# taconite/IntrinsicAvatar

Measured on AMD Instinct MI355X. Metric: rays/sec (fwd+bwd) at 540×540, 1024 spp; fraction of HBM / MFMA roofline, higher is better.
Workload: dtype f32

## Files before the change

include/ia_amd.h:

```cpp
#ifndef IA_AMD_H
#define IA_AMD_H

#include <stdint.h>

#ifdef __cplusplus
extern "C" {
#endif

#define IA_OK 0
#define IA_ERR_INVALID (-1)
#define IA_ERR_LAUNCH (-2)
#define IA_ERR_UNSUPPORTED (-3)

typedef void* ia_stream_t;

int ia_version(void);
const char* ia_last_error(void);

int64_t ia_scan_tmp_bytes(int64_t n);
int ia_exclusive_scan_i64(const int64_t* in, int64_t* out, int64_t* total, int64_t n, void* tmp, ia_stream_t stream);
int ia_exclusive_scan_i32(const int32_t* in, int32_t* out, int32_t* total, int64_t n, void* tmp, ia_stream_t stream);

int ia_occgrid_pack_bits(const uint8_t* binaries, int64_t n_cells, uint32_t* bits, ia_stream_t stream);

// ... 55 lines not shown
int ia_ray_resampling(int64_t n_rays, int64_t n_in, int n, const int32_t* packed_info, const float* starts, const float* ends,
                      const float* weights, const float* sdfs, const int32_t* resample_packed_info, int64_t n_out,
                      float* resample_ts, float* resample_offsets, int64_t* surface_idx,
                      int64_t* resample_indices, int32_t* resample_fg_counts, int32_t* resample_bg_counts, void* tmp,
                      ia_stream_t stream);
int ia_ray_resampling_upto(int64_t n_rays, int64_t n_in, int n, const int32_t* packed_info, const float* starts, const float* ends,
                           const float* weights, const float* sdfs, const int32_t* resample_packed_info, int64_t n_out,
                           const int32_t* n_out_dev, float* resample_ts, float* resample_offsets, int64_t* surface_idx,
                           int64_t* resample_indices, int32_t* resample_fg_counts, int32_t* resample_bg_counts, void* tmp,
                           ia_stream_t stream);
int ia_ray_resampling_merge(int64_t n_rays, int64_t n_in, int n, const int32_t* packed_info, const float* vals,
                            const uint8_t* is_left, const uint8_t* is_right, const float* weights,
                            const int32_t* resample_packed_info, float* resample_vals, float* resample_dists,
                            uint8_t* resample_is_left, uint8_t* resample_is_right, uint8_t* is_resample,
                            uint8_t* is_fg_sample, void* tmp, ia_stream_t stream);
int ia_ray_resampling_merge_count(int64_t n_rays, int64_t n_in, int n, const int32_t* packed_info, const float* vals,
                                  const uint8_t* is_left, const uint8_t* is_right, const float* weights, int32_t* cnt,
                                  int32_t* start, int32_t* total, void* tmp, void* scan_tmp, ia_stream_t stream);
int ia_ray_resampling_merge_fill(int64_t n_rays, int64_t n_in, int n, const int32_t* packed_info, const float* vals,
                                 const uint8_t* is_left, const uint8_t* is_right, const int32_t* cnt, const int32_t* start,
                                 float* out_vals, uint8_t* out_is_left, uint8_t* out_is_right, int64_t* out_ray_indices,
                                 int32_t* out_packed_info, void* tmp, ia_stream_t stream);
int ia_ray_resampling_fine(int64_t n_rays, int64_t n_in, int n, const int32_t* packed_info, const float* starts, const float* ends,
                           const float* weights, const int32_t* resample_packed_info, int64_t n_out, float* resample_starts,
                           float* resample_ends, uint8_t* is_fg_sample, void* tmp, ia_stream_t stream);
int ia_ray_resampling_sdf_fine(int64_t n_rays, int64_t n_in, int n, const int32_t* packed_info, const float* starts,
                               const float* ends, const float* alphas, const float* sdfs,
                               const int32_t* resample_packed_info, int64_t n_out, float* resample_starts,
                               float* resample_ends, uint8_t* is_fg_sample, void* tmp, ia_stream_t stream);

int ia_fg_count(int64_t n_rays, const int32_t* resampled_packed_info, const uint8_t* is_fg, int32_t* cnt, int32_t* start, int32_t* total,
                void* scan_tmp, ia_stream_t stream);
int ia_fg_compact(int64_t n_rays, const int32_t* resampled_packed_info, const uint8_t* is_fg, const float* starts, const float* ends,
                  const int32_t* cnt, const int32_t* start, int64_t* ray_indices, float* t_starts, float* t_ends, int32_t* out_packed_info,
                  ia_stream_t stream);

int ia_interval_samples_count(int64_t n_edges, const uint8_t* is_left, int32_t* pos, int32_t* total, void* scan_tmp, ia_stream_t stream);
int ia_interval_samples_count_upto(int64_t capacity, const uint8_t* is_left, const int32_t* n_edges, int32_t* pos, int32_t* total,
                                   void* scan_tmp, ia_stream_t stream);
int ia_interval_samples_fill(int64_t n_rays, int64_t n_edges, const int32_t* edge_packed_info, const float* vals,
                             const int64_t* ray_indices, const uint8_t* is_left, const int32_t* pos, const int32_t* total,
                             int64_t* left_idx, float* t_starts, float* t_ends, int64_t* sample_ray_indices,
                             int32_t* sample_packed_info, ia_stream_t stream);
int ia_samples_to_edges(int64_t n_edges, const uint8_t* is_left, const int32_t* pos, const float* sample_vals, float fill, float* out,
                        ia_stream_t stream);

#define IA_LAYOUT_NCDHW 0
#define IA_LAYOUT_NDHWC 1
int ia_precompute(int B, int D, int H, int W, const float* voxel_w , const float* tfs ,
                  const float* offset , const float* scale ,
                  float* voxel_d , float* voxel_J ,
                  float* voxel_J_cl , ia_stream_t stream);
int ia_fuse_broyden(int B, int64_t N, int I, const float* xd_tgt , const float* voxel_J, int layout,
                    int D, int H, int W, const float* tfs, const int32_t* bone_ids ,
                    const float* offset, const float* scale, float cvg_threshold, float dvg_threshold,
                    float* x , float* J_inv , uint8_t* is_valid ,
                    float* fwd_J ,
                    ia_stream_t stream);
int ia_filter(int64_t N, int I, const float* x , const uint8_t* mask, uint8_t* out, ia_stream_t stream);
int ia_cell_tightness(int D, int H, int W, const float* voxel_J_cl , const float* offset, const float* scale, float tau,
                      uint8_t* cell_tight , ia_stream_t stream);
int ia_fuse_broyden_spec(int64_t N, int I, const float* xd_tgt , const float* voxel_J_cl , int D, int H, int W,
                         const float* tfs , const int32_t* bone_ids, const float* offset, const float* scale,
                         float cvg_threshold, float dvg_threshold, float eps, float* x , float* J_inv ,
                         uint8_t* is_valid , float* fwd_J , uint64_t* counters,
                         const uint8_t* cell_tight , ia_stream_t stream);
int ia_spec_rows_slots(void);
size_t ia_spec_rows_overflow_bytes(int64_t N);
int64_t ia_spec_rows_overflow_capacity(int64_t N);
int ia_fuse_broyden_spec_rows(int64_t N, int I, const float* xd_tgt, const float* voxel_J_cl, int D, int H, int W, const float* tfs,
                              const int32_t* bone_ids, const float* offset, const float* scale, float cvg_threshold,
                              float dvg_threshold, float eps, float* x_rows, float* J_inv, float* fwd_J, int32_t* cnt, uint32_t* meta,
                              int32_t* start, int32_t* ovf_head, void* ovf_scratch, int32_t* total_and_overflow, void* scan_tmp,
                              uint64_t* counters, const int32_t* order ,
                              const uint8_t* cell_tight , ia_stream_t stream);
int ia_deform_rows_pack(int64_t N, int I, const float* x_rows, const int32_t* cnt, const uint32_t* meta, const int32_t* start,
                        const int32_t* ovf_head, const void* ovf_scratch, float* cand_x, int32_t* cand_src,
                        const float* norm_center , const float* norm_scale ,
                        ia_stream_t stream);
int64_t ia_deform_rows_pack_split_tmp_bytes(int64_t N);
int ia_deform_rows_pack_split(int64_t N, int I, const float* x_rows, const int32_t* cnt, const uint32_t* meta, const int32_t* start,
                              const int32_t* ovf_head, const void* ovf_scratch, int32_t* first_pos, int32_t* first_tile_off, int32_t* n_first,
                              float* cand_x, const float* norm_center, const float* norm_scale, void* scan_tmp, ia_stream_t stream);
int ia_deform_select_min_split(int64_t P, const int32_t* start, const int32_t* cnt, const int32_t* first_pos, const int32_t* first_tile_off,
                               const int32_t* n_first, const float* cand_sdf, const int32_t* order, float* sdf, ia_stream_t stream);
int ia_broyden_stats(int B, int64_t N, int I, const float* xd_tgt, const float* voxel_J, int layout, int D, int H, int W,
                     const float* tfs, const int32_t* bone_ids, const float* offset, const float* scale,
                     float cvg_threshold, float dvg_threshold, uint64_t* counters, ia_stream_t stream);
int ia_broyden_voxel_stats(int64_t N, int I, int init_major, const float* xd_tgt, const float* voxel_J , int D, int H,
                           int W, const float* tfs, const int32_t* bone_ids, const float* offset, const float* scale,
                           uint64_t* counters, ia_stream_t stream);

int64_t ia_hashgrid_n_entries(int n_levels, int log2_hashmap_size, int base_resolution, float per_level_scale);
int ia_hashgrid_fwd(int64_t n, const float* x , const float* params, int n_levels, int n_features,
                    int log2_hashmap_size, int base_resolution, float per_level_scale,
                    float* out, int out_stride, float* dy_dx , ia_stream_t stream);
int64_t ia_hashgrid_fwd_scratch_bytes(int64_t n, int n_levels, int with_jac);
int ia_hashgrid_fwd_xcd(int64_t n, const float* x, const float* params, int n_levels, int n_features,
                        int log2_hashmap_size, int base_resolution, float per_level_scale, float* out, int out_stride,
                        float* dy_dx, void* scratch, ia_stream_t stream);
int ia_hashgrid_bwd(int64_t n, const float* x, int n_levels, int n_features, int log2_hashmap_size,
                    int base_resolution, float per_level_scale, const float* g_enc ,
                    int g_enc_stride, const float* g_jac , int g_jac_stride, const float* q ,
                    float* grad_params, ia_stream_t stream);
int64_t ia_hashgrid_bwd_scratch_bytes(int64_t n, int n_levels, int log2_hashmap_size, int base_resolution,
                                      float per_level_scale);
int ia_hashgrid_bwd_binned(int64_t n, const float* x, int n_levels, int n_features, int log2_hashmap_size,
                           int base_resolution, float per_level_scale, const float* g_enc, int g_enc_stride,
                           const float* g_jac, int g_jac_stride, const float* q, float* grad_params,
                           uint32_t level_mask ,
                           void* scratch, int64_t scratch_bytes, ia_stream_t stream);
int ia_hashgrid_jac_contract(int mode, int64_t n, int K, const float* jac, const float* v, int v_stride, float* out,
                             int out_stride, ia_stream_t stream);
int ia_sh4_fwd(int64_t n, const float* d01, float* out, int out_stride, ia_stream_t stream);

int ia_mlp_fwd(int kind, int64_t n, int n_segs, const float* const* seg_ptr, const int* seg_stride,
               const int* seg_width, const float* seg_mul, const float* seg_add,
               const float* W1, const float* b1, const float* W2, const float* b2, const float* Wo, const float* bo,
               float* y, int y_stride, const float* jac, int xyz_col, const float* inv_scale_host, float* grad,
               ia_stream_t stream);

int ia_deform_filter_count(int64_t P, int I, const float* x , const uint8_t* valid ,
                           uint8_t* mask , int32_t* cnt , ia_stream_t stream);
int ia_deform_compact(int64_t P, int I, const float* x, const uint8_t* mask, const int32_t* start,
                      float* cand_x , int32_t* cand_src , ia_stream_t stream);
size_t ia_deform_filter_compact_tmp_bytes(int64_t P);
int ia_deform_filter_compact(int64_t P, int I, const float* x, const uint8_t* valid, int32_t* cnt , int32_t* start ,
                             float* cand_x , int32_t* cand_src , uint8_t* mask ,
                             int32_t* total , void* tmp, size_t tmp_bytes, ia_stream_t stream);
size_t ia_deform_filter_tiles_tmp_bytes(int64_t P);
int ia_deform_filter_tiles(int64_t P, int I, float* x, const uint8_t* valid, int32_t* cnt, int32_t* start, int32_t* src_local ,
                           uint8_t* mask , int32_t* total, void* tmp, size_t tmp_bytes, ia_stream_t stream);
int ia_deform_pack_tiles(int64_t P, int I, const float* x, const int32_t* src_local , int32_t* start, float* cand_x,
                         int32_t* cand_src , const void* tmp, ia_stream_t stream);
int ia_deform_select(int64_t P, const int32_t* start, const int32_t* cnt, const float* cand_x,
                     const int32_t* cand_src, const float* cand_sdf, int sdf_stride, const float* cand_grad ,
                     const float* cand_feat , int feat_stride, int feat_dim, const float* c2w ,
                     float* pts_cano , float* sdf , uint8_t* valid , int32_t* sel ,
                     float* grad_posed , float* grad_cano , float* feat ,
                     ia_stream_t stream);
int ia_ray_points(int64_t n, const float* rays_o, const float* rays_d, const int64_t* ray_indices,
                  const float* t0, const float* t1, float* pts, ia_stream_t stream);
int ia_shade_prep(int64_t n, const float* sdf_grad , const float* rays_d, const int64_t* ray_indices,
                  const float* w2s_rot , float* normal_smpl, float* normal_world, float* refl01,
                  ia_stream_t stream);
int ia_laplace_alpha(int64_t n, const float* sdf, const float* dists, float dist_const, const float* beta,
                     float* alpha, ia_stream_t stream);
int ia_laplace_alpha_intervals(int64_t n, const float* sdf, const float* t_starts, const float* t_ends, const float* beta, float* alpha,
                               ia_stream_t stream);
int ia_laplace_alpha_bwd(int64_t n, const float* sdf, const float* dists, float dist_const, const float* beta,
                         const float* g_alpha, float* g_sdf, float* g_beta , ia_stream_t stream);

int ia_sh4_bwd(int64_t n, const float* d01, const float* g_sh, int g_stride, float* g_d01, ia_stream_t stream);
int ia_shade_prep_bwd(int64_t n, const float* sdf_grad, const float* rays_d, const int64_t* ray_indices,
                      const float* w2s_rot, const float* g_normal_world , const float* g_refl01 ,
                      const float* g_normal_smpl , float* g_sdf_grad, ia_stream_t stream);
int ia_mlp_bwd(int kind, int64_t n, int n_segs, const float* const* seg_ptr, const int* seg_stride,
               const int* seg_width, const float* seg_mul, const float* seg_add,
               const float* W1, const float* b1, const float* W2, const float* b2, const float* Wo, const float* bo,
               const float* g_y , float* g_x, int gx_stride,
               float* X , float* A1 , float* A2 ,
               float* G1 , float* G2 , float* G3 , ia_stream_t stream);
int ia_sdf_mlp_bwd(int64_t n, int n_segs, const float* const* seg_ptr, const int* seg_stride, const int* seg_width,
                   const float* seg_mul, const float* seg_add, const float* W1, const float* b1, const float* Wo,
                   const float* bo, const float* jac, const float* g_out, const float* q, float* gE, float* gG,
                   float* Hh , float* U , float* DZ , float* GZ ,
// ... 30 lines not shown
                     int env_h, int env_w, const float* w2s_rot, const float* g_Lo, const float* g_Lo_diff,
                     const float* g_Lo_spec, float* g_normal, float* g_albedo, float* g_roughness, float* g_metallic,
                     float* g_env_base, void* scratch , size_t scratch_bytes, ia_stream_t stream);
size_t ia_pbr_shade_bwd_scratch_bytes(int64_t F);
int ia_brdf_sample(int64_t F, const float* normal, const float* view_dirs, const float* roughness, const float* u,
                   float* out_dirs, ia_stream_t stream);
int ia_brdf_pdf(int64_t F, const float* normal, const float* view_dirs, const float* out_dirs, const float* roughness,
                float* pdf, ia_stream_t stream);
int ia_envlight_eval(int64_t n, const float* dirs_world, const float* env_base, const float* env_pmf, int env_h,
                     int env_w, float* rgb , float* pdf , ia_stream_t stream);

int ia_occgrid_ema(int64_t n_cells, float* occs, const float* occ_new, float ema_decay, ia_stream_t stream);
int64_t ia_occgrid_tmp_bytes(int res_x, int res_y, int res_z);
int ia_occgrid_binarize(int res_x, int res_y, int res_z, const float* occs, float thre_max, int keep_largest_component,
                        uint8_t* binaries, float* thre_out, void* tmp, ia_stream_t stream);

int ia_select_push(int64_t n, const float* out13, const float* grad_c, const uint8_t* valid, const float* fwd_J,
                   const int32_t* cand_src, const int32_t* sel, float* feat, float* sdf, float* sdf_grad, float* c2w,
                   ia_stream_t stream);
int ia_select_push_bwd(int64_t n, const uint8_t* valid, const float* c2w, const float* g_feat, const float* g_sdf,
                       const float* g_sdf_grad, float* g_out13, float* g_grad_c, ia_stream_t stream);
int64_t ia_eikonal_partials(int64_t n);
int ia_eikonal(int64_t n, const float* sdf_grad, const uint8_t* valid, float* partial, ia_stream_t stream);
int ia_eikonal_bwd(int64_t n, const float* sdf_grad, const uint8_t* valid, const float* weight, float* g_sdf_grad,
                   ia_stream_t stream);

int ia_adam_step(int n_tensors, float* const* params, const float* const* grads, float* const* exp_avg,
                 float* const* exp_avg_sq, const int64_t* numel, const float* step_size, const float* weight_decay,
                 float beta1, float beta2, float eps, float bias_correction2_sqrt, float grad_scale, ia_stream_t stream);

int ia_vi_layout(int64_t n_rays, int spp, const int32_t* resampled_packed_info, const int32_t* bg_counts, int32_t* fg_ray_cnt,
                 ia_stream_t stream);
int ia_vi_gather(int64_t n_rays, const int32_t* resampled_packed_info, const int32_t* fg_ray_cnt, const int32_t* fg_start,
                 const float* ts , const int64_t* sampled_idx , const int32_t* fg_counts ,
                 const float* weights , const float* rays_o, const float* rays_d, const float* normals ,
                 const float* albedo , const float* roughness , const float* metallic ,
                 int32_t* fg_src , int32_t* fg_ray , float* positions , float* view_dirs ,
                 float* o_normals, float* o_albedo, float* o_roughness, float* o_metallic, float* o_weights ,
                 ia_stream_t stream);
int ia_vi_gather_bwd(int64_t S, const int32_t* fg_counts, const int32_t* fg_off, const float* g_normals_fg,
                     const float* g_albedo_fg, const float* g_roughness_fg, const float* g_metallic_fg,
                     const float* g_weights_fg, float* g_normals, float* g_albedo, float* g_roughness, float* g_metallic,
                     float* g_weights, ia_stream_t stream);
int ia_vi_composite(int64_t n_rays, const int32_t* resampled_packed_info, const int32_t* fg_ray_cnt, const int32_t* fg_start,
                    const int32_t* bg_counts, const float* weights_fg, const float* Lo , const float* transmittance ,
                    const float* background , const float* background_rays, float* rgb , ia_stream_t stream);
int ia_vi_composite_bwd(int64_t n_rays, int64_t F, const int32_t* resampled_packed_info, const int32_t* bg_counts,
                        const int32_t* fg_ray, const float* weights_fg, const float* Lo, const float* background,
                        const float* background_rays , const float* g_rgb, float* g_weights_fg,
                        float* g_Lo, float* g_transmittance, ia_stream_t stream);
int ia_vi_indices(int64_t n_rays, int spp, const int32_t* resampled_packed_info, const int32_t* fg_ray_cnt,
                  const int32_t* fg_start, const int32_t* bg_counts, const int64_t* sampled_idx, const int32_t* fg_counts,
                  const float* weights, const float* transmittance, int64_t* fg_indices, int64_t* bg_indices,
                  int64_t* ray_indices, float* resampled_weights, ia_stream_t stream);
int ia_light_shuffle(int64_t n_rays, int spp, const int32_t* fg_ray_cnt, const int32_t* fg_start, const float* u ,
                     int32_t* shuffled , ia_stream_t stream);
int ia_envlight_sample(int64_t k, const float* u , const double* cdf , int env_h, int env_w, const float* rot,
                       float* dirs , ia_stream_t stream);
int ia_secondary_mask(int64_t F, const float* normals, const float* dirs, const int32_t* dir_index, int32_t* flag,
                      ia_stream_t stream);
int ia_secondary_compact(int64_t F, const int32_t* flag, const int32_t* slot, const float* positions, const float* dirs,
                         const int32_t* dir_index, float* rays_o, float* rays_d, int32_t* src, float* dense_dirs ,
                         ia_stream_t stream);
int ia_secondary_scatter(int64_t M, const int32_t* src, const float* transmittance, const float* rgb, float* dense_transmittance,
                         float* dense_rgb, ia_stream_t stream);
int ia_secondary_gather_dense(int64_t F, const int32_t* flag, const int32_t* slot, const float* transmittance, const float* rgb,
                              float* dense_transmittance, float* dense_rgb, ia_stream_t stream);

int ia_scatterer_sample(int64_t F, int lobes, const float* normal, const float* wi, const float* alpha, const float* u ,
                        float* wo, ia_stream_t stream);
int ia_scatterer_pdf(int64_t F, int lobes, const float* normal, const float* wi, const float* wo, const float* alpha, float* pdf,
                     ia_stream_t stream);
int ia_scatterer_eval(int64_t F, int lobes, const float* normal, const float* wi, const float* wo, const float* alpha,
                      const float* albedo, const float* metallic, float* diff, float* spec, ia_stream_t stream);

int ia_morton_keys(int64_t n, const float* pts , const float* origin_host3 , float inv_cell,
                   int32_t* keys, ia_stream_t stream);
int ia_gather_rows3(int64_t n, const float* src, const int64_t* order, float* dst, ia_stream_t stream);
int ia_scatter_f32(int64_t n, const float* src, const int64_t* order, float* dst, ia_stream_t stream);
int ia_sort_rank_mode(void);
size_t ia_morton_order_tmp_bytes(int64_t n);
int ia_morton_order(int64_t n, const float* pts , const float* origin_host3, float inv_cell, int drop_bits,
                    int32_t* order , void* tmp, size_t tmp_bytes, ia_stream_t stream);
int ia_gather_rows3_i32(int64_t n, const float* src, const int32_t* order, float* dst, ia_stream_t stream);
int ia_scatter_f32_i32(int64_t n, const float* src, const int32_t* order, float* dst, ia_stream_t stream);
int ia_scatter_rows3_i32(int64_t n, const float* src , const int32_t* order, float* dst ,
                         ia_stream_t stream);

int ia_gaussian_histogram(int64_t n, const float* x, const float* sigma, int bins, float vmin, float vmax, float* out,
                          ia_stream_t stream);
int ia_gaussian_histogram_bwd(int64_t n, const float* x, const float* sigma, int bins, float vmin, float vmax, const float* g_out,
                              float* g_x, float* g_sigma, ia_stream_t stream);

int ia_sdf_levels_fwd(int64_t n, const void* levels, const float* xp , const float* W1 ,
                      const float* b1, const float* Wo , const float* bo, float* sdf ,
                      ia_stream_t stream);
int64_t ia_hashgrid_fwd_levels_jac_offset(int64_t n, int n_levels);
int ia_hashgrid_fwd_levels(int64_t n, const float* x, const float* params, int n_levels, int n_features, int log2_hashmap_size,
                           int base_resolution, float per_level_scale, int with_jac, void* scratch, ia_stream_t stream);
int ia_sdf_levels_fwd_grad(int64_t n, const void* levels, const float* levels_jac, const float* xp, const float* W1, const float* b1,
                           const float* Wo , const float* bo, float* y, int y_stride, const float* inv_scale_host,
                           float* grad, ia_stream_t stream);
int ia_deform_select_min(int64_t P, const int32_t* start, const int32_t* cnt, const float* cand_sdf, float* sdf, ia_stream_t stream);
int ia_deform_select_min_scatter(int64_t P, const int32_t* start, const int32_t* cnt, const float* cand_sdf, const int32_t* order,
                                 float* sdf, ia_stream_t stream);

int ia_normalize_points(int64_t n, const float* x, const float* center, const float* scale, float* out, ia_stream_t stream);
int ia_effective_weights(int mode, int M, int N, const float* g, const float* v, const int* src, const float* mul, float* out,
                         ia_stream_t stream);
int ia_effective_weights_bwd(int mode, int M, int N, const float* g, const float* v, const int* src, const float* mul, const float* g_out,
                             float* g_v, float* g_g, ia_stream_t stream);
int ia_sg_image(int K, int H, int W, const float* axis, const float* log_lambda, const float* mu, float* out, ia_stream_t stream);
int64_t ia_sg_image_bwd_tmp_bytes(int K);
int ia_sg_image_bwd(int K, int H, int W, const float* axis, const float* log_lambda, const float* mu, const float* g_img, void* tmp,
                    float* g_axis, float* g_log_lambda, float* g_mu, ia_stream_t stream);
int64_t ia_envlight_pdf_tables_tmp_bytes(int H, int W);
int ia_envlight_pdf_tables(int H, int W, const float* base, float* pmf, double* cdf, void* tmp, ia_stream_t stream);
int ia_uniform_sphere_stratified(int n_theta, int n_phi, const float* u, float* dirs, float* inv_pdf, ia_stream_t stream);
int ia_material_affine(int64_t n, const float* m, float albedo_scale, float albedo_bias, float roughness_scale, float roughness_bias,
                       float metallic_scale, float metallic_bias, float* albedo, float* roughness, float* metallic, ia_stream_t stream);
int ia_material_affine_bwd(int64_t n, const float* g_albedo, const float* g_roughness, const float* g_metallic, float albedo_scale,
                           float roughness_scale, float metallic_scale, float* g_m, ia_stream_t stream);
int64_t ia_phys_loss_tmp_bytes(int64_t n);
int ia_phys_loss(int64_t n, const float* comp_rgb, const float* comp_rgb_phys, const float* opacity, const float* target_rgb,
                 const float* target_mask, const float* eik_partials, int eik_k, float lambda_phys, float lambda_mask, float lambda_eik,
                 float eik_denom, float* terms, void* tmp , ia_stream_t stream);
int ia_phys_loss_bwd(int64_t n, const float* comp_rgb, const float* comp_rgb_phys, const float* opacity, const float* target_rgb,
                     const float* target_mask, const float* g_loss, float lambda_phys, float lambda_mask, float lambda_eik, float eik_denom,
                     float* g_comp_rgb, float* g_comp_rgb_phys, float* g_opacity, float* g_eik_sum, ia_stream_t stream);
int ia_edge_min_sdf(int64_t n_edges, const float* sdf, const uint8_t* is_left, float* out, ia_stream_t stream);
int ia_transform_rays_w2s(int64_t n, const float* rays, int ray_stride, const float* w2s, int variant, float* out, ia_stream_t stream);

int64_t ia_mc_scratch_bytes(int nx, int ny, int nz);
int ia_mc_count(int nx, int ny, int nz, const float* level, float threshold, void* scratch, int64_t* totals, ia_stream_t stream);
int ia_mc_emit(int nx, int ny, int nz, const float* level, float threshold, const float* box, const void* scratch, int32_t* first_vid,
               float* v_pos, int64_t* t_pos_idx, ia_stream_t stream);
int ia_mc_grid_points(int64_t n, int64_t start, int nx, int ny, int nz, const float* axes, const float* center, const float* scale,
                      float* out, ia_stream_t stream);

int64_t ia_metric_tmp_bytes(void);
int ia_metric_sq_err(int64_t n, int C, const float* a, const float* b, const uint8_t* mask, void* tmp, double* sums, float* psnr,
                     ia_stream_t stream);
int ia_metric_albedo_sums(int64_t n, const float* gt, const float* pred, const uint8_t* mask, void* tmp, double* sums, float* ratio,
                          ia_stream_t stream);
int ia_metric_albedo_apply(int64_t n, const float* pred, const uint8_t* mask, const float* ratio, float* out, ia_stream_t stream);
int ia_metric_transform_normals(int64_t n, const float* normals, const float* w2c_rot, float* out, ia_stream_t stream);
int ia_metric_normal_error(int64_t n, const float* pred, const float* target, const uint8_t* mask, const float* w2c_rot, int transform,
                           int normalize, float* cam_out, float* err_map, void* tmp, double* sums, float* result, ia_stream_t stream);
int ia_metric_mask_rect(int H, int W, const uint8_t* mask, void* tmp, int32_t* rect, ia_stream_t stream);
int64_t ia_metric_ssim_tmp_bytes(int H, int W, int C);
int ia_metric_ssim(int H, int W, int C, const float* a, const float* b, const int32_t* rect, void* tmp, double* out, ia_stream_t stream);

int ia_knn_points(int64_t P, int V, int K, const float* p1, const float* p2, float* d2, int32_t* idx, ia_stream_t stream);
int ia_skin_blend(int64_t P, int V, int K, const float* d2, const int32_t* idx, const float* weights, float* out, ia_stream_t stream);
int ia_skin_smooth(int D, int H, int W, const float* src, float* dst, ia_stream_t stream);
int ia_skin_grid_points(int D, int H, int W, float ratio, float scale, float ox, float oy, float oz, float* out, ia_stream_t stream);

int ia_make_rays(int64_t n, const int64_t* pixels, int H, int W, const double* cam_host, float* rays_o, float* rays_d, ia_stream_t stream);
int ia_window_minmax(int64_t outer, int64_t len, int64_t inner, int k, const float* in, float* out_min, float* out_max, ia_stream_t stream);
int64_t ia_flag_lists_scratch_bytes(int64_t F, int64_t N);
int ia_flag_lists_count(int64_t F, int64_t N, const float* mask, const float* mask_i, const float* mask_o, void* scratch, int32_t* totals,
                        ia_stream_t stream);
int ia_flag_lists_fill(int64_t F, int64_t N, const float* mask, const float* mask_i, const float* mask_o, const void* scratch,
                       const int32_t* totals, int32_t* mask_start, int32_t* edge_start, int32_t* counts, int32_t* mask_loc, int32_t* edge_loc,
                       ia_stream_t stream);
int ia_sample_batch(int64_t n, int64_t num_mask, int64_t num_edge, int64_t frame, int64_t F, int H, int W, const int64_t* words,
// ... 9 lines not shown
```

intrinsicavatar_amd/csrc/deform.hip:

```cpp
#include "ia_common.h"

namespace {

constexpr int THREADS = 256;

constexpr int FC_MAX_I = 16;
__global__ __launch_bounds__(THREADS) void filter_count_kernel(int64_t P, int I, const float* __restrict__ x,
                                                                const uint8_t* __restrict__ valid,
                                                                uint8_t* __restrict__ mask, int32_t* __restrict__ cnt)
{
    extern __shared__ __attribute__((aligned(16))) float s_x[];
    uint8_t* s_v = reinterpret_cast<uint8_t*>(s_x + THREADS * I * 3);
    const int64_t p0 = (int64_t)blockIdx.x * THREADS;
    const int rows = (int)((P - p0) < THREADS ? (P - p0) : THREADS);
    const int nf = rows * I * 3, nb = rows * I;
    const float* gx = x + p0 * I * 3;
    const uint8_t* gv = valid + p0 * I;
    if ((reinterpret_cast<uintptr_t>(gx) & 15) == 0) {
        const float4* g4 = reinterpret_cast<const float4*>(gx);
        float4* s4 = reinterpret_cast<float4*>(s_x);
        for (int i = threadIdx.x; i < nf / 4; i += THREADS) s4[i] = g4[i];
        for (int i = (nf / 4) * 4 + threadIdx.x; i < nf; i += THREADS) s_x[i] = gx[i];
    } else {
        for (int i = threadIdx.x; i < nf; i += THREADS) s_x[i] = gx[i];
    }
    for (int i = threadIdx.x; i < nb; i += THREADS) s_v[i] = gv[i];
    __syncthreads();
    const int t = threadIdx.x;
    const bool live = t < rows;
    const float* xr = s_x + t * I * 3;
    const uint8_t* vr = s_v + t * I;
    int c = 0;
    unsigned keep_bits = 0;
    for (int i = 0; live && i < I; i++) {
        bool keep = vr[i] != 0;
        if (keep) {
            const float xi0 = xr[i * 3 + 0], xi1 = xr[i * 3 + 1], xi2 = xr[i * 3 + 2];
            for (int j = i + 1; j < I; j++) {
                if (!vr[j]) continue;
                const float d0 = xi0 - xr[j * 3 + 0];
                const float d1 = xi1 - xr[j * 3 + 1];
                const float d2 = xi2 - xr[j * 3 + 2];
                const float dist = d0 * d0 + d1 * d1 + d2 * d2;
                if ((double)dist < 0.0001 * 0.0001) { keep = false; break; }
            }
        }
        keep_bits |= (keep ? 1u : 0u) << i;
        c += keep ? 1 : 0;
    }
    if (live) cnt[p0 + t] = c;
    __syncthreads();
    for (int i = 0; live && i < I; i++) s_v[t * I + i] = (keep_bits >> i) & 1u;
    __syncthreads();
    uint8_t* gm = mask + p0 * I;
    for (int i = threadIdx.x; i < nb; i += THREADS) gm[i] = s_v[i];
}

__global__ __launch_bounds__(THREADS) void compact_fill_kernel(int64_t P, int I, const float* __restrict__ x,
                                                                const uint8_t* __restrict__ mask,
                                                                const int32_t* __restrict__ start,
                                                                float* __restrict__ cand_x, int32_t* __restrict__ cand_src)
{
    const int64_t p = (int64_t)blockIdx.x * THREADS + threadIdx.x;
    if (p >= P) return;
    int q = start[p];
    for (int i = 0; i < I; i++) {
        if (!mask[p * I + i]) continue;
        cand_x[(int64_t)q * 3 + 0] = x[(p * I + i) * 3 + 0];
        cand_x[(int64_t)q * 3 + 1] = x[(p * I + i) * 3 + 1];
        cand_x[(int64_t)q * 3 + 2] = x[(p * I + i) * 3 + 2];
        cand_src[q] = (int32_t)(p * I + i);
        q++;
    }
}

constexpr int FCC_ROWS = 256, FCC_LOOK = 4;
constexpr uint64_t FCC_AGGREGATE = 1ull << 32, FCC_PREFIX = 2ull << 32;

template <int IT, bool LOCAL>
__global__ __launch_bounds__(FCC_ROWS) void filter_compact_kernel(int64_t P, int I_rt, uint32_t magic_I, int n_tiles, const float* x,
                                                                  const uint8_t* __restrict__ valid, uint64_t* desc,
                                                                  int32_t* __restrict__ cnt, int32_t* __restrict__ start, float* cand_x,
                                                                  int32_t* __restrict__ cand_src, uint8_t* __restrict__ mask,
// ... 202 lines not shown
    for (int j = 0; j < c; j++) {
        const float v = cand_sdf[s + j];
        if (v < best) best = v;
    }
    sdf_out[dst] = best;
}

__global__ __launch_bounds__(THREADS) void select_min_split_kernel(int64_t P, const int32_t* __restrict__ start, const int32_t* __restrict__ cnt,
                                                                    const int32_t* __restrict__ first_pos, const int32_t* __restrict__ first_tile_off,
                                                                    const int32_t* __restrict__ n_first, const float* __restrict__ cand_sdf,
                                                                    const int32_t* __restrict__ order, float* __restrict__ sdf_out)
{
    const int64_t p = (int64_t)blockIdx.x * THREADS + threadIdx.x;
    if (p >= P) return;
    const int c = cnt[p];
    const int64_t dst = order ? (int64_t)order[p] : p;
    float best = 1e5f;
    if (c > 0) {
        const int64_t fp = (int64_t)first_pos[p] + first_tile_off[p >> 10];
        const float v0 = cand_sdf[fp];
        if (v0 < best) best = v0;
        const int64_t tail = (int64_t)*n_first + ((int64_t)start[p] - fp) - 1;
        for (int j = 1; j < c; j++) {
            const float v = cand_sdf[tail + j];
            if (v < best) best = v;
        }
    }
    sdf_out[dst] = best;
}

__global__ __launch_bounds__(THREADS) void select_kernel(
    int64_t P, const int32_t* __restrict__ start, const int32_t* __restrict__ cnt, const float* __restrict__ cand_x,
    const int32_t* __restrict__ cand_src, const float* __restrict__ cand_sdf, int sdf_stride,
    const float* __restrict__ cand_grad, const float* __restrict__ cand_feat, int feat_stride, int feat_dim,
    const float* __restrict__ c2w , float* __restrict__ pts_cano, float* __restrict__ sdf_out,
    uint8_t* __restrict__ valid_out, int32_t* __restrict__ sel_out, float* __restrict__ grad_posed,
    float* __restrict__ grad_cano, float* __restrict__ feat_out)
{
    const int64_t p = (int64_t)blockIdx.x * THREADS + threadIdx.x;
    if (p >= P) return;
    const int s = start[p], c = cnt[p];
    float best = 1e5f;
    int bq = -1;
    for (int j = 0; j < c; j++) {
        const float v = cand_sdf[(int64_t)(s + j) * sdf_stride];
        if (v < best) { best = v; bq = s + j; }
    }
    sdf_out[p] = best;
    valid_out[p] = c > 0 ? 1 : 0;
    if (sel_out) sel_out[p] = bq;
    if (bq >= 0) {
        pts_cano[p * 3 + 0] = cand_x[(int64_t)bq * 3 + 0];
        pts_cano[p * 3 + 1] = cand_x[(int64_t)bq * 3 + 1];
        pts_cano[p * 3 + 2] = cand_x[(int64_t)bq * 3 + 2];
    } else {
        pts_cano[p * 3 + 0] = 0.f; pts_cano[p * 3 + 1] = 0.f; pts_cano[p * 3 + 2] = 0.f;
    }
    if (grad_posed) {
        float g0 = 0.f, g1 = 0.f, g2 = 1.f;
        float h0 = 0.f, h1 = 0.f, h2 = 1.f;
        if (bq >= 0) {
            h0 = cand_grad[(int64_t)bq * 3 + 0]; h1 = cand_grad[(int64_t)bq * 3 + 1]; h2 = cand_grad[(int64_t)bq * 3 + 2];
            const float* R = c2w + (int64_t)cand_src[bq] * 9;
            g0 = R[0] * h0 + R[1] * h1 + R[2] * h2;
            g1 = R[3] * h0 + R[4] * h1 + R[5] * h2;
            g2 = R[6] * h0 + R[7] * h1 + R[8] * h2;
        }
        grad_posed[p * 3 + 0] = g0; grad_posed[p * 3 + 1] = g1; grad_posed[p * 3 + 2] = g2;
        if (grad_cano) { grad_cano[p * 3 + 0] = h0; grad_cano[p * 3 + 1] = h1; grad_cano[p * 3 + 2] = h2; }
    }
    if (feat_out)
        for (int k = 0; k < feat_dim; k++)
            feat_out[p * feat_dim + k] = bq >= 0 ? cand_feat[(int64_t)bq * feat_stride + k] : 0.0f;
}

__global__ __launch_bounds__(THREADS) void ray_points_kernel(int64_t n, const float* __restrict__ rays_o,
                                                              const float* __restrict__ rays_d,
                                                              const int64_t* __restrict__ ray_indices,
                                                              const float* __restrict__ t0, const float* __restrict__ t1,
                                                              float* __restrict__ pts)
{
    const int64_t i = (int64_t)blockIdx.x * THREADS + threadIdx.x;
    if (i >= n) return;
    const int64_t r = ray_indices[i];
    const float t = t1 ? (t0[i] + t1[i]) / 2.0f : t0[i];
    pts[i * 3 + 0] = rays_o[r * 3 + 0] + rays_d[r * 3 + 0] * t;
    pts[i * 3 + 1] = rays_o[r * 3 + 1] + rays_d[r * 3 + 1] * t;
    pts[i * 3 + 2] = rays_o[r * 3 + 2] + rays_d[r * 3 + 2] * t;
}

__device__ __forceinline__ void normalize3(float v[3], float eps)
{
    const float n = sqrtf(v[0] * v[0] + v[1] * v[1] + v[2] * v[2]);
    const float d = fmaxf(n, eps);
    v[0] /= d; v[1] /= d; v[2] /= d;
}

__global__ __launch_bounds__(THREADS) void shade_prep_kernel(int64_t n, const float* __restrict__ sdf_grad,
                                                              const float* __restrict__ rays_d,
                                                              const int64_t* __restrict__ ray_indices,
                                                              const float* __restrict__ R, float* __restrict__ normal_smpl,
                                                              float* __restrict__ normal_world, float* __restrict__ refl01)
{
    const int64_t i = (int64_t)blockIdx.x * THREADS + threadIdx.x;
    if (i >= n) return;
    const int64_t r = ray_indices[i];
    float g[3] = {sdf_grad[i * 3 + 0], sdf_grad[i * 3 + 1], sdf_grad[i * 3 + 2]};
    float d[3] = {rays_d[r * 3 + 0], rays_d[r * 3 + 1], rays_d[r * 3 + 2]};
    float nw[3], vw[3];
#pragma unroll
    for (int c = 0; c < 3; c++) {
        nw[c] = g[0] * R[0 * 3 + c] + g[1] * R[1 * 3 + c] + g[2] * R[2 * 3 + c];
        vw[c] = d[0] * R[0 * 3 + c] + d[1] * R[1 * 3 + c] + d[2] * R[2 * 3 + c];
    }
    normalize3(nw, 1e-6f);
    normalize3(vw, 1e-6f);
    normalize3(g, 1e-6f);
    const float dt = -(vw[0] * nw[0] + vw[1] * nw[1] + vw[2] * nw[2]);
#pragma unroll
    for (int c = 0; c < 3; c++) {
        normal_smpl[i * 3 + c] = g[c];
        normal_world[i * 3 + c] = nw[c];
        refl01[i * 3 + c] = ((2.0f * dt * nw[c] + vw[c]) + 1.0f) / 2.0f;
    }
}

__global__ __launch_bounds__(THREADS) void shade_prep_bwd_kernel(int64_t n, const float* __restrict__ sdf_grad,
                                                                  const float* __restrict__ rays_d,
                                                                  const int64_t* __restrict__ ray_indices,
                                                                  const float* __restrict__ R, const float* __restrict__ g_nw,
                                                                  const float* __restrict__ g_refl01, const float* __restrict__ g_ns,
                                                                  float* __restrict__ g_sdf_grad)
{
    const int64_t i = (int64_t)blockIdx.x * THREADS + threadIdx.x;
    if (i >= n) return;
    const int64_t r = ray_indices[i];
    const float g[3] = {sdf_grad[i * 3 + 0], sdf_grad[i * 3 + 1], sdf_grad[i * 3 + 2]};
    const float d[3] = {rays_d[r * 3 + 0], rays_d[r * 3 + 1], rays_d[r * 3 + 2]};
    float nwu[3], vw[3], nw[3];
#pragma unroll
    for (int c = 0; c < 3; c++) {
        nwu[c] = g[0] * R[0 * 3 + c] + g[1] * R[1 * 3 + c] + g[2] * R[2 * 3 + c];
        vw[c] = d[0] * R[0 * 3 + c] + d[1] * R[1 * 3 + c] + d[2] * R[2 * 3 + c];
    }
    normalize3(vw, 1e-6f);
    const float len = sqrtf(nwu[0] * nwu[0] + nwu[1] * nwu[1] + nwu[2] * nwu[2]);
    const float den = fmaxf(len, 1e-6f);
#pragma unroll
    for (int c = 0; c < 3; c++) nw[c] = nwu[c] / den;
    const float dt = -(vw[0] * nw[0] + vw[1] * nw[1] + vw[2] * nw[2]);
    float G[3];
    float gr_dot_nw = 0.f;
#pragma unroll
    for (int c = 0; c < 3; c++) gr_dot_nw += 0.5f * (g_refl01 ? g_refl01[i * 3 + c] : 0.f) * nw[c];
#pragma unroll
    for (int c = 0; c < 3; c++)
        G[c] = (g_nw ? g_nw[i * 3 + c] : 0.f) + 2.0f * dt * 0.5f * (g_refl01 ? g_refl01[i * 3 + c] : 0.f) - 2.0f * gr_dot_nw * vw[c];
    float Gu[3];
    if (len > 1e-6f) {
        const float dn = nw[0] * G[0] + nw[1] * G[1] + nw[2] * G[2];
#pragma unroll
        for (int c = 0; c < 3; c++) Gu[c] = (G[c] - nw[c] * dn) / len;
    } else {
#pragma unroll
        for (int c = 0; c < 3; c++) Gu[c] = G[c] / 1e-6f;
    }
    float gs[3] = {0.f, 0.f, 0.f};
    if (g_ns) {
        const float nrm = fmaxf(sqrtf(g[0] * g[0] + g[1] * g[1] + g[2] * g[2]), 1e-6f);
        const float ns[3] = {g[0] / nrm, g[1] / nrm, g[2] / nrm};
        const float dsn = g_ns[i * 3 + 0] * ns[0] + g_ns[i * 3 + 1] * ns[1] + g_ns[i * 3 + 2] * ns[2];
// ... 457 lines not shown
```

intrinsicavatar_amd/csrc/snarf.hip:

```cpp
#include <stdlib.h>

#include "ia_common.h"
#include "ia_zero.h"

namespace {

constexpr int THREADS = 256;

__global__ __launch_bounds__(THREADS) void precompute_kernel(int B, int D, int H, int W,
                                                              const float* __restrict__ voxel_w,
                                                              const float* __restrict__ tfs,
                                                              const float* __restrict__ offset,
                                                              const float* __restrict__ scale,
                                                              float* __restrict__ voxel_d, float* __restrict__ voxel_J,
                                                              float* __restrict__ voxel_J_cl)
{
    __shared__ float s_tfs[24 * 12];
    const int64_t vol = (int64_t)D * H * W;
    const int idx_b = blockIdx.y;
    for (int t = threadIdx.x; t < 24 * 12; t += THREADS) {
        const int j = t / 12, c = t % 12;
        s_tfs[t] = tfs[((int64_t)idx_b * 24 + j) * 16 + c];
    }
    __syncthreads();
// ... 983 lines not shown
                m |= (uint32_t)i << (8 * kept);
            } else {
                const int q = atomicAdd(ovf_count, 1);
                if (q < ovf_cap) {
                    ovf_rec[3 * q + 0] = (int32_t)p; ovf_rec[3 * q + 1] = i; ovf_rec[3 * q + 2] = last;
                    ovf_x[3 * q + 0] = fx[3 * i]; ovf_x[3 * q + 1] = fx[3 * i + 1]; ovf_x[3 * q + 2] = fx[3 * i + 2];
                    ovf_keep[q] = 1;
                    last = q;
                }
            }
            kept++;
        }
        cnt[p] = kept;
        meta[p] = m | (last >= 0 ? 0x80000000u : 0u);
        if (last >= 0) ovf_head[p] = last;
    }
}

constexpr int FIRST_TILE_PACK = 1024;
__global__ __launch_bounds__(THREADS) void rows_pack_kernel(int64_t N, int I, const float* __restrict__ x, const int32_t* __restrict__ cnt,
                                                             const uint32_t* __restrict__ meta, const int32_t* __restrict__ start,
                                                             const int32_t* __restrict__ ovf_head, const int32_t* __restrict__ ovf_rec,
                                                             const float* __restrict__ ovf_x, const uint8_t* __restrict__ ovf_keep,
                                                             float* __restrict__ cand_x, int32_t* __restrict__ cand_src,
                                                             const float* __restrict__ nc, const float* __restrict__ ns,
                                                             const int32_t* __restrict__ first_pos = nullptr, const int32_t* __restrict__ first_tile_off = nullptr,
                                                             const int32_t* __restrict__ n_first = nullptr)
{
    const int64_t p = (int64_t)blockIdx.x * THREADS + threadIdx.x;
    if (p >= N) return;
    int c = cnt[p];
    if (c == 0) return;
    const bool nrm = nc != nullptr;
    const float c0 = nrm ? nc[0] : 0.f, c1 = nrm ? nc[1] : 0.f, c2 = nrm ? nc[2] : 0.f;
    const float s0 = nrm ? ns[0] : 1.f, s1 = nrm ? ns[1] : 1.f, s2 = nrm ? ns[2] : 1.f;
    auto put = [&](int64_t q_, float a, float b, float d) {
        if (nrm) { a = (a - c0) / s0 + 0.5f; b = (b - c1) / s1 + 0.5f; d = (d - c2) / s2 + 0.5f; }
        cand_x[q_ * 3 + 0] = a; cand_x[q_ * 3 + 1] = b; cand_x[q_ * 3 + 2] = d;
    };
    const int64_t st = start[p];
    const int64_t fp = first_pos ? (int64_t)first_pos[p] + first_tile_off[p / FIRST_TILE_PACK] : 0, tail = first_pos ? (int64_t)*n_first + (st - fp) - 1 : 0;
    auto pos = [&](int j) -> int64_t { return first_pos ? (j == 0 ? fp : tail + j) : st + j; };
    int j = 0;
    const unsigned m = meta[p];
    if (m & 0x80000000u) {
        for (int k = ovf_head[p]; k >= 0; k = ovf_rec[3 * k + 2]) {
            if (!ovf_keep[k]) continue;
            const int64_t q = pos(j);
            put(q, ovf_x[3 * k], ovf_x[3 * k + 1], ovf_x[3 * k + 2]);
            if (cand_src) cand_src[q] = (int32_t)(p * I + ovf_rec[3 * k + 1]);
            j++;
        }
        c -= j;
    }
    const float* row = x + p * (SPEC_ROOTS * 3);
    for (int k = 0; k < c; k++) {
        const int slot = c - 1 - k;
        const int64_t q = pos(j + k);
        put(q, row[slot * 3 + 0], row[slot * 3 + 1], row[slot * 3 + 2]);
        if (cand_src) cand_src[q] = (int32_t)(p * I + ((m >> (8 * slot)) & 0xffu));
    }
}

constexpr int FIRST_TILE = 1024;
__global__ __launch_bounds__(256) void first_scan_tiles_kernel(int64_t N, const int32_t* __restrict__ cnt, int32_t* __restrict__ first_local,
                                                                int32_t* __restrict__ tile_sums)
{
    __shared__ int s_w[4];
    const int lane = threadIdx.x & 63, wave = threadIdx.x >> 6;
    const int64_t base = (int64_t)blockIdx.x * FIRST_TILE + (int64_t)threadIdx.x * 4;
    int v[4], local = 0;
#pragma unroll
    for (int k = 0; k < 4; k++) { v[k] = (base + k < N && cnt[base + k] > 0) ? 1 : 0; local += v[k]; }
    int inc = local;
#pragma unroll
    for (int off = 1; off < 64; off <<= 1) { const int o = __shfl_up(inc, off, 64); if (lane >= off) inc += o; }
    if (lane == 63) s_w[wave] = inc;
    __syncthreads();
    int run = inc - local;
    for (int w = 0; w < wave; w++) run += s_w[w];
#pragma unroll
    for (int k = 0; k < 4; k++) { if (base + k < N) first_local[base + k] = run; run += v[k]; }
    if (threadIdx.x == 255) tile_sums[blockIdx.x] = run;
}

template <int LAYOUT>
__global__ __launch_bounds__(THREADS) void broyden_stats_kernel(
    int64_t total, int64_t N, int I, const float* __restrict__ xd_tgt, const float* __restrict__ voxel_J, int D, int H,
    int W, const float* __restrict__ tfs, const int32_t* __restrict__ bone_ids, const float* __restrict__ offset_g,
    const float* __restrict__ scale_g, float cvg_threshold, float dvg_threshold, unsigned long long* __restrict__ counters)
{
    const int64_t index = (int64_t)blockIdx.x * THREADS + threadIdx.x;
    unsigned fetches = 0, corners = 0, outcome = 3;
    if (index < total) {
        const int64_t vol = (int64_t)D * H * W;
        const int i_batch = (int)(index / (N * I));
        const int64_t i_point = (index % (N * I)) / I;
        const int i_init = (int)((index % (N * I)) % I);
        const float* vJ = (LAYOUT == IA_LAYOUT_NDHWC) ? voxel_J : voxel_J + (int64_t)i_batch * 12 * vol;
        const int vox0 = (LAYOUT == IA_LAYOUT_NDHWC) ? (int)(i_batch * vol) : 0;
        const float offset[3] = {offset_g[0], offset_g[1], offset_g[2]};
        const float scale[3] = {scale_g[0], scale_g[1], scale_g[2]};
        auto in_range_corners = [&](float gx, float gy, float gz) -> unsigned {
            float ix = ((gx + 1.f) / 2) * (W - 1), iy = ((gy + 1.f) / 2) * (H - 1), iz = ((gz + 1.f) / 2) * (D - 1);
            if (ix > 2147483646.0f || ix < -2147483648.0f || !isfinite(ix)) ix = -100.0f;
            if (iy > 2147483646.0f || iy < -2147483648.0f || !isfinite(iy)) iy = -100.0f;
            if (iz > 2147483646.0f || iz < -2147483648.0f || !isfinite(iz)) iz = -100.0f;
            const int x0 = (int)floorf(ix), y0 = (int)floorf(iy), z0 = (int)floorf(iz);
            const unsigned cx = (unsigned)(x0 >= 0 && x0 < W) + (unsigned)(x0 + 1 >= 0 && x0 + 1 < W);
            const unsigned cy = (unsigned)(y0 >= 0 && y0 < H) + (unsigned)(y0 + 1 >= 0 && y0 + 1 < H);
            const unsigned cz = (unsigned)(z0 >= 0 && z0 < D) + (unsigned)(z0 + 1 >= 0 && z0 + 1 < D);
            return cx * cy * cz;
        };
        float gx[3], gx_new[3] = {0, 0, 0}, xt[3], x_l[3];
        xt[0] = xd_tgt[((int64_t)i_batch * N + i_point) * 3 + 0];
        xt[1] = xd_tgt[((int64_t)i_batch * N + i_point) * 3 + 1];
        xt[2] = xd_tgt[((int64_t)i_batch * N + i_point) * 3 + 2];
        const float* T = tfs + ((int64_t)i_batch * 24 + bone_ids[i_init]) * 16;
        const float ixd = xt[0] - T[0 * 4 + 3], iyd = xt[1] - T[1 * 4 + 3], izd = xt[2] - T[2 * 4 + 3];
        x_l[0] = ixd * T[0 * 4 + 0] + iyd * T[1 * 4 + 0] + izd * T[2 * 4 + 0];
        x_l[1] = ixd * T[0 * 4 + 1] + iyd * T[1 * 4 + 1] + izd * T[2 * 4 + 1];
        x_l[2] = ixd * T[0 * 4 + 2] + iyd * T[1 * 4 + 2] + izd * T[2 * 4 + 2];
        float Jl[12];
        {
            const float a = scale[0] * (x_l[0] + offset[0]), b = scale[1] * (x_l[1] + offset[1]), c = scale[2] * (x_l[2] + offset[2]);
            grid_sample_J<LAYOUT>(vJ, vox0, D, H, W, a, b, c, Jl);
            fetches++; corners += in_range_corners(a, b, c);
        }
        float Ji[9];
        Ji[0] = Jl[0]; Ji[3] = Jl[1]; Ji[6] = Jl[2];
        Ji[1] = Jl[4]; Ji[4] = Jl[5]; Ji[7] = Jl[6];
        Ji[2] = Jl[8]; Ji[5] = Jl[9]; Ji[8] = Jl[10];
        outcome = 2;
        for (int it = 0; it < 10; it++) {
            if (it == 0) {
                gx[0] = Jl[0] * x_l[0] + Jl[1] * x_l[1] + Jl[2] * x_l[2] + Jl[3];
                gx[1] = Jl[4] * x_l[0] + Jl[5] * x_l[1] + Jl[6] * x_l[2] + Jl[7];
                gx[2] = Jl[8] * x_l[0] + Jl[9] * x_l[1] + Jl[10] * x_l[2] + Jl[11];
                gx[0] = gx[0] - xt[0]; gx[1] = gx[1] - xt[1]; gx[2] = gx[2] - xt[2];
            } else {
                gx[0] = gx_new[0]; gx[1] = gx_new[1]; gx[2] = gx_new[2];
            }
            const float u0 = -Ji[0] * gx[0] + -Ji[1] * gx[1] + -Ji[2] * gx[2];
            const float u1 = -Ji[3] * gx[0] + -Ji[4] * gx[1] + -Ji[5] * gx[2];
            const float u2 = -Ji[6] * gx[0] + -Ji[7] * gx[1] + -Ji[8] * gx[2];
            x_l[0] += u0; x_l[1] += u1; x_l[2] += u2;
            const float ix = scale[0] * (x_l[0] + offset[0]);
            const float iy = scale[1] * (x_l[1] + offset[1]);
            const float iz = scale[2] * (x_l[2] + offset[2]);
            grid_sample_J<LAYOUT>(vJ, vox0, D, H, W, ix, iy, iz, Jl);
            fetches++; corners += in_range_corners(ix, iy, iz);
            gx_new[0] = Jl[0] * x_l[0] + Jl[1] * x_l[1] + Jl[2] * x_l[2] + Jl[3] - xt[0];
            gx_new[1] = Jl[4] * x_l[0] + Jl[5] * x_l[1] + Jl[6] * x_l[2] + Jl[7] - xt[1];
            gx_new[2] = Jl[8] * x_l[0] + Jl[9] * x_l[1] + Jl[10] * x_l[2] + Jl[11] - xt[2];
            const float norm_gx = gx_new[0] * gx_new[0] + gx_new[1] * gx_new[1] + gx_new[2] * gx_new[2];
            if (norm_gx < cvg_threshold * cvg_threshold) {
                outcome = (ix >= -1 && ix <= 1 && iy >= -1 && iy <= 1 && iz >= -1 && iz <= 1) ? 0 : 1;
                break;
            } else if (norm_gx > dvg_threshold * dvg_threshold) {
                outcome = 1;
                break;
            }
            J_inv_update(Ji, u0, u1, u2, gx_new[0] - gx[0], gx_new[1] - gx[1], gx_new[2] - gx[2]);
        }
    }
    unsigned f = fetches, c = corners;
// ... 311 lines not shown
#undef IA_SPEC_LAUNCH_S
    return ia::check_launch(what);
}

IA_EXPORT int ia_fuse_broyden_spec(int64_t N, int I, const float* xd_tgt, const float* voxel_J_cl, int D, int H, int W, const float* tfs,
                                   const int32_t* bone_ids, const float* offset, const float* scale, float cvg_threshold,
                                   float dvg_threshold, float eps, float* x, float* J_inv, uint8_t* is_valid, float* fwd_J,
                                   uint64_t* counters, const uint8_t* cell_tight, ia_stream_t stream)
{
    SpecFlag none = {nullptr, nullptr, nullptr, nullptr, 0};
    return launch_spec(false, N, I, xd_tgt, voxel_J_cl, D, H, W, tfs, bone_ids, offset, scale, cvg_threshold, dvg_threshold, eps, x, J_inv,
                       is_valid, fwd_J, counters, nullptr, nullptr, none, nullptr, cell_tight, stream, "ia_fuse_broyden_spec");
}

IA_EXPORT int ia_spec_rows_slots(void) { return SPEC_ROOTS; }

extern "C" int ia_exclusive_scan_i32(const int32_t* in, int32_t* out, int32_t* total, int64_t n, void* tmp, ia_stream_t stream);

static const int SPEC_OVF_CAP = 1 << 18;

struct OvfLayout { int32_t* count; int32_t* rec; float* x; uint8_t* keep; SpecFlag flag; };
static size_t ovf_layout(void* scratch, int64_t N, OvfLayout* L)
{
    const size_t fcap = (size_t)spec_flag_cap(N);
    ia::Carver c(scratch);
    L->count = c.take<int32_t>(2, 64);
    L->rec = c.take<int32_t>((size_t)SPEC_OVF_CAP * 3, 64);
    L->x = c.take<float>((size_t)SPEC_OVF_CAP * 3, 64);
    L->keep = c.take<uint8_t>((size_t)SPEC_OVF_CAP, 64);
    c.skip(64);
    L->flag.count = L->count ? L->count + 1 : nullptr;
    L->flag.point = c.take<int32_t>(fcap, 64);
    L->flag.valid = c.take<uint32_t>(fcap, 64);
    L->flag.x = c.take<float>(fcap * 16 * 3, 64);
    c.skip(64);
    L->flag.cap = (int)fcap;
    return c.need(8);
}

IA_EXPORT size_t ia_spec_rows_overflow_bytes(int64_t N)
{
    OvfLayout L;
    return ovf_layout(nullptr, N, &L);
}

struct PackSplitTmp {
    int32_t* sums;
    void* scan_tmp;
    int64_t tiles;
};
static size_t pack_split_layout(void* tmp, int64_t N, PackSplitTmp* t)
{
    t->tiles = (N + FIRST_TILE - 1) / FIRST_TILE;
    ia::Carver c(tmp);
    t->sums = c.take<int32_t>((size_t)t->tiles);
    t->scan_tmp = c.take<char>((size_t)ia_scan_tmp_bytes(t->tiles));
    c.skip(1024);
    return c.need(8);
}

IA_EXPORT int64_t ia_deform_rows_pack_split_tmp_bytes(int64_t N)
{
    PackSplitTmp t;
    return (int64_t)pack_split_layout(nullptr, N > 0 ? N : 0, &t);
}

__global__ void rows_report_kernel(const int32_t* __restrict__ counts, int flag_cap, int32_t* __restrict__ out)
{
    if (threadIdx.x == 0 && blockIdx.x == 0) out[0] = counts[0] > SPEC_OVF_CAP ? flag_cap + 1 : counts[1];
}

IA_EXPORT int ia_fuse_broyden_spec_rows(int64_t N, int I, const float* xd_tgt, const float* voxel_J_cl, int D, int H, int W, const float* tfs,
                                        const int32_t* bone_ids, const float* offset, const float* scale, float cvg_threshold,
                                        float dvg_threshold, float eps, float* x_rows, float* J_inv, float* fwd_J, int32_t* cnt,
                                        uint32_t* meta, int32_t* start, int32_t* ovf_head, void* ovf_scratch, int32_t* total_and_overflow,
                                        void* scan_tmp, uint64_t* counters, const int32_t* order, const uint8_t* cell_tight, ia_stream_t stream)
{
    IA_REQUIRE(N * I < ((int64_t)1 << 31), "ia_fuse_broyden_spec_rows: N * I must stay below 2^31");
    hipStream_t s = (hipStream_t)stream;
    OvfLayout o;
    ovf_layout(ovf_scratch, N, &o);
    ia::zero_bytes(o.count, 2 * sizeof(int32_t), s);
    if (N == 0) {
        ia::zero_bytes(total_and_overflow, 2 * sizeof(int32_t), s);
        return ia::check_launch("ia_fuse_broyden_spec_rows");
    }
    int64_t small_max = (int64_t)1 << 18;
    if (const char* e = getenv("IA_BR_SMALL_MAX")) { small_max = atoll(e); if (small_max > ((int64_t)1 << 18)) small_max = (int64_t)1 << 18; }
    const bool small = N <= small_max && N <= o.flag.cap && I <= 16 && counters == nullptr;
    int r;
    if (small) {
        IA_REQUIRE(I >= 1 && I <= 16, "ia_fuse_broyden_spec_rows: 1 <= I <= 16 inits");
        IA_REQUIRE((int64_t)D * H * W < ((int64_t)1 << 26), "voxel grid too large for 32-bit byte offsets (48 B per voxel)");
        ia::zero_bytes(o.flag.valid, (size_t)N * sizeof(uint32_t), s);
        broyden_items_rows_kernel<<<ia::cdiv(N * I, THREADS), THREADS, 0, s>>>(N, I, xd_tgt, voxel_J_cl, D, H, W, tfs, bone_ids, offset, scale,
                                                                              cvg_threshold, dvg_threshold, J_inv, fwd_J, o.flag, order);
        r = ia::check_launch("ia_fuse_broyden_spec_rows(items)");
    } else {
        r = launch_spec(true, N, I, xd_tgt, voxel_J_cl, D, H, W, tfs, bone_ids, offset, scale, cvg_threshold, dvg_threshold, eps, x_rows,
                        J_inv, nullptr, fwd_J, counters, cnt, meta, o.flag, order, cell_tight, stream, "ia_fuse_broyden_spec_rows");
    }
    if (r != IA_OK) return r;
    rows_flagged_kernel<<<(small ? (int)ia::cdiv(N, THREADS) : 64), THREADS, 0, s>>>(o.flag, I, x_rows, cnt, meta, o.count, SPEC_OVF_CAP, ovf_head,
                                                                                    o.rec, o.x, o.keep);
    r = ia::check_launch("ia_fuse_broyden_spec_rows(flagged)");
    if (r != IA_OK) return r;
    if (small) zero_i32_kernel<<<1, 64, 0, s>>>(o.flag.count);
    r = ia_exclusive_scan_i32(cnt, start, total_and_overflow, N, scan_tmp, stream);
    if (r != IA_OK) return r;
    rows_report_kernel<<<1, 64, 0, s>>>(o.count, o.flag.cap, total_and_overflow + 1);
    return ia::check_launch("ia_fuse_broyden_spec_rows(report)");
}

IA_EXPORT int64_t ia_spec_rows_overflow_capacity(int64_t N) { return spec_flag_cap(N); }

IA_EXPORT int ia_deform_rows_pack(int64_t N, int I, const float* x_rows, const int32_t* cnt, const uint32_t* meta, const int32_t* start,
                                  const int32_t* ovf_head, const void* ovf_scratch, float* cand_x, int32_t* cand_src,
                                  const float* norm_center, const float* norm_scale, ia_stream_t stream)
{
    if (N == 0) return IA_OK;
    IA_REQUIRE(cand_x != x_rows, "ia_deform_rows_pack: cand_x must not alias x_rows");
    IA_REQUIRE((norm_center == nullptr) == (norm_scale == nullptr), "ia_deform_rows_pack: norm_center and norm_scale go together");
    OvfLayout o;
    ovf_layout(const_cast<void*>(ovf_scratch), N, &o);
    rows_pack_kernel<<<ia::cdiv(N, THREADS), THREADS, 0, (hipStream_t)stream>>>(N, I, x_rows, cnt, meta, start, ovf_head, o.rec, o.x, o.keep,
                                                                                cand_x, cand_src, norm_center, norm_scale);
    return ia::check_launch("ia_deform_rows_pack");
}

IA_EXPORT int ia_deform_rows_pack_split(int64_t N, int I, const float* x_rows, const int32_t* cnt, const uint32_t* meta, const int32_t* start,
                                        const int32_t* ovf_head, const void* ovf_scratch, int32_t* first_pos, int32_t* first_tile_off,
                                        int32_t* n_first, float* cand_x, const float* norm_center, const float* norm_scale, void* scan_tmp,
                                        ia_stream_t stream)
{
    if (N == 0) return IA_OK;
    static_assert(FIRST_TILE == FIRST_TILE_PACK, "one tile size");
    IA_REQUIRE(cand_x != x_rows, "ia_deform_rows_pack_split: cand_x must not alias x_rows");
    IA_REQUIRE((norm_center == nullptr) == (norm_scale == nullptr), "ia_deform_rows_pack_split: norm_center and norm_scale go together");
    IA_REQUIRE(first_pos != nullptr && first_tile_off != nullptr && n_first != nullptr && scan_tmp != nullptr,
               "ia_deform_rows_pack_split: first_pos, first_tile_off, n_first and scan_tmp are required");
    hipStream_t s = (hipStream_t)stream;
    PackSplitTmp t;
    pack_split_layout(scan_tmp, N, &t);
    const int64_t tiles = t.tiles;
    int32_t* sums = t.sums;
    void* tmp = t.scan_tmp;
    first_scan_tiles_kernel<<<(int)tiles, 256, 0, s>>>(N, cnt, first_pos, sums);
    const int r = ia_exclusive_scan_i32(sums, first_tile_off, n_first, tiles, tmp, stream);
    if (r != IA_OK) return r;
    OvfLayout o;
    ovf_layout(const_cast<void*>(ovf_scratch), N, &o);
    rows_pack_kernel<<<ia::cdiv(N, THREADS), THREADS, 0, s>>>(N, I, x_rows, cnt, meta, start, ovf_head, o.rec, o.x, o.keep, cand_x, nullptr,
                                                              norm_center, norm_scale, first_pos, first_tile_off, n_first);
    return ia::check_launch("ia_deform_rows_pack_split");
}

IA_EXPORT int ia_filter(int64_t N, int I, const float* x, const uint8_t* mask, uint8_t* out, ia_stream_t stream)
{
    if (N == 0) return IA_OK;
    filter_kernel<<<ia::cdiv(N, THREADS), THREADS, 0, (hipStream_t)stream>>>(N, I, x, mask, out);
    return ia::check_launch("ia_filter");
}

IA_EXPORT int ia_broyden_stats(int B, int64_t N, int I, const float* xd_tgt, const float* voxel_J, int layout, int D, int H,
                               int W, const float* tfs, const int32_t* bone_ids, const float* offset, const float* scale,
                               float cvg_threshold, float dvg_threshold, uint64_t* counters ,
                               ia_stream_t stream)
{
    const int64_t total = (int64_t)B * N * I;
    if (total == 0) return IA_OK;
    IA_REQUIRE(layout == IA_LAYOUT_NCDHW || layout == IA_LAYOUT_NDHWC, "unknown voxel_J layout");
    IA_REQUIRE((int64_t)B * D * H * W < ((int64_t)1 << 26), "voxel grid too large for 32-bit byte offsets");
    const int grid = ia::cdiv(total, THREADS);
    unsigned long long* c = reinterpret_cast<unsigned long long*>(counters);
    if (layout == IA_LAYOUT_NDHWC)
        broyden_stats_kernel<IA_LAYOUT_NDHWC><<<grid, THREADS, 0, (hipStream_t)stream>>>(
            total, N, I, xd_tgt, voxel_J, D, H, W, tfs, bone_ids, offset, scale, cvg_threshold, dvg_threshold, c);
    else
        broyden_stats_kernel<IA_LAYOUT_NCDHW><<<grid, THREADS, 0, (hipStream_t)stream>>>(
            total, N, I, xd_tgt, voxel_J, D, H, W, tfs, bone_ids, offset, scale, cvg_threshold, dvg_threshold, c);
    return ia::check_launch("ia_broyden_stats");
}

IA_EXPORT int ia_broyden_voxel_stats(int64_t N, int I, int init_major, const float* xd_tgt, const float* voxel_J, int D, int H, int W,
                                     const float* tfs, const int32_t* bone_ids, const float* offset, const float* scale,
                                     uint64_t* counters, ia_stream_t stream)
{
    if (N == 0) return IA_OK;
    const int64_t total = ((N + 63) / 64) * 64 * I;
    broyden_voxel_stats_kernel<<<ia::cdiv(total, THREADS), THREADS, 0, (hipStream_t)stream>>>(
        N, I, init_major, xd_tgt, voxel_J, D, H, W, tfs, bone_ids, offset, scale, reinterpret_cast<unsigned long long*>(counters));
    return ia::check_launch("ia_broyden_voxel_stats");
}
```

intrinsicavatar_amd/csrc/sort.hip:

```cpp
#include <cstdlib>
#include <cstring>
#include <mutex>

#include "ia_common.h"

namespace {

constexpr int THREADS = 256;

__device__ __forceinline__ uint32_t spread10(uint32_t v)
{
    v &= 0x3FFu;
    v = (v | (v << 16)) & 0x030000FFu;
    v = (v | (v << 8)) & 0x0300F00Fu;
    v = (v | (v << 4)) & 0x030C30C3u;
    return (v | (v << 2)) & 0x09249249u;
}

__global__ __launch_bounds__(THREADS) void gather_rows3_i32_kernel(int64_t n, const float* __restrict__ src, const int32_t* __restrict__ order,
                                                                    float* __restrict__ dst)
{
    const int64_t i = (int64_t)blockIdx.x * THREADS + threadIdx.x;
    if (i >= n) return;
    const int64_t j = order[i];
    dst[3 * i] = src[3 * j]; dst[3 * i + 1] = src[3 * j + 1]; dst[3 * i + 2] = src[3 * j + 2];
}

__global__ __launch_bounds__(THREADS) void scatter_f32_i32_kernel(int64_t n, const float* __restrict__ src, const int32_t* __restrict__ order,
                                                                   float* __restrict__ dst)
{
    const int64_t i = (int64_t)blockIdx.x * THREADS + threadIdx.x;
    if (i >= n) return;
    dst[order[i]] = src[i];
}

__global__ __launch_bounds__(THREADS) void scatter_rows3_i32_kernel(int64_t n, const float* __restrict__ src, const int32_t* __restrict__ order,
                                                                     float* __restrict__ dst)
{
    const int64_t i = (int64_t)blockIdx.x * THREADS + threadIdx.x;
    if (i >= n) return;
    const int64_t j = order[i];
    dst[3 * j] = src[3 * i]; dst[3 * j + 1] = src[3 * i + 1]; dst[3 * j + 2] = src[3 * i + 2];
}

#ifndef IA_SORT_THREADS
#define IA_SORT_THREADS 512
#endif
constexpr int ST = IA_SORT_THREADS;
constexpr int SW = ST / 64;
constexpr int SI = 32;
constexpr int TILE = ST * SI;
constexpr int SEG = 64 * SI;
#ifndef IA_SORT_BITS
#define IA_SORT_BITS 10
#endif
constexpr int MAXB = IA_SORT_BITS;
constexpr int NBMAX = 1 << MAXB;
constexpr int CT = 256;
constexpr int CI = TILE / CT;

__device__ __forceinline__ uint32_t morton_key(const float* __restrict__ pts, int64_t i, float ox, float oy, float oz, float inv_cell, int raster = 0)
{
    const float fx = (pts[3 * i] - ox) * inv_cell, fy = (pts[3 * i + 1] - oy) * inv_cell, fz = (pts[3 * i + 2] - oz) * inv_cell;
    const uint32_t x = (uint32_t)fminf(fmaxf(fx, 0.0f), 1023.0f), y = (uint32_t)fminf(fmaxf(fy, 0.0f), 1023.0f),
                   z = (uint32_t)fminf(fmaxf(fz, 0.0f), 1023.0f);
    if (raster > 0) {
        const uint32_t m = (1u << raster) - 1u;
        const uint32_t hi = spread10(x >> raster) | (spread10(y >> raster) << 1) | (spread10(z >> raster) << 2);
        return (hi << (3 * raster)) | ((z & m) << (2 * raster)) | ((y & m) << raster) | (x & m);
    }
    return spread10(x) | (spread10(y) << 1) | (spread10(z) << 2);
}

__device__ __forceinline__ uint64_t digit_peers(uint32_t digit, int bits, bool valid)
{
    uint64_t peers = __ballot(valid);
    for (int b = 0; b < bits; b++) {
        const bool bit = (digit >> b) & 1u;
        const uint64_t m = __ballot(bit);
        peers &= bit ? m : ~m;
    }
    return peers;
}

template <bool FIRST>
__global__ __launch_bounds__(CT) void radix_count_kernel(int64_t n, const float* __restrict__ pts, float ox, float oy, float oz, float inv_cell,
                                                          uint32_t* __restrict__ keys , const uint2* __restrict__ pairs ,
                                                          int shift, int bits, int32_t* __restrict__ hist, int ntiles, int raster)
{
    __shared__ int32_t s_hist[NBMAX];
    const int nb = 1 << bits;
    const uint32_t mask = (uint32_t)nb - 1u;
    for (int d = threadIdx.x; d < nb; d += CT) s_hist[d] = 0;
    __syncthreads();
    const int lane = threadIdx.x & 63;
    const int64_t base = (int64_t)blockIdx.x * TILE + threadIdx.x;
    for (int r0 = 0; r0 < CI; r0 += 8) {
        uint32_t key[8];
#pragma unroll
        for (int r = 0; r < 8; r++) {
            const int64_t i = base + (int64_t)(r0 + r) * CT;
            key[r] = 0;
            if (i < n) {
                if (FIRST) { key[r] = morton_key(pts, i, ox, oy, oz, inv_cell, raster); keys[i] = key[r]; }
                else key[r] = pairs[i].x;
            }
        }
#pragma unroll
        for (int r = 0; r < 8; r++) {
            const bool valid = base + (int64_t)(r0 + r) * CT < n;
            const uint32_t digit = (key[r] >> shift) & mask;
            const uint64_t vm = __ballot(valid);
            if (vm == 0ull) continue;
            const uint32_t d0 = __builtin_amdgcn_readlane(digit, __ffsll((long long)vm) - 1);
            if (__ballot(valid && digit != d0) == 0ull) {
                if (lane == __ffsll((long long)vm) - 1) atomicAdd(&s_hist[d0], __popcll(vm));
            } else if (valid) {
                atomicAdd(&s_hist[digit], 1);
            }
        }
    }
    __syncthreads();
    for (int d = threadIdx.x; d < nb; d += CT) hist[(int64_t)blockIdx.x * nb + d] = s_hist[d];
}

constexpr int SCAN_CHUNK = 64;

__global__ __launch_bounds__(256) void radix_chunk_sums_kernel(const int32_t* __restrict__ hist, int nb, int ntiles, int32_t* __restrict__ chunk_sum)
{
    const int t0 = blockIdx.x * SCAN_CHUNK, t1 = min(t0 + SCAN_CHUNK, ntiles);
    for (int d = threadIdx.x; d < nb; d += 256) {
        int32_t acc = 0;
#pragma unroll 8
        for (int t = t0; t < t1; t++) acc += hist[(int64_t)t * nb + d];
        chunk_sum[(int64_t)blockIdx.x * nb + d] = acc;
    }
}

__global__ __launch_bounds__(1024) void radix_chunk_bases_kernel(const int32_t* __restrict__ chunk_sum, int nb, int nchunks,
                                                                 int32_t* __restrict__ chunk_off, int32_t* __restrict__ digit_base)
{
    __shared__ int32_t s_w[16];
    const int d = threadIdx.x, lane = d & 63, wave = d >> 6;
    int32_t total = 0;
    if (d < nb) {
#pragma unroll 8
        for (int c = 0; c < nchunks; c++) {
            const int32_t v = chunk_sum[(int64_t)c * nb + d];
            chunk_off[(int64_t)c * nb + d] = total;
            total += v;
        }
    }
    int32_t inc = total;
#pragma unroll
    for (int off = 1; off < 64; off <<= 1) {
        const int32_t o = __shfl_up(inc, off, 64);
        if (lane >= off) inc += o;
    }
    if (lane == 63) s_w[wave] = inc;
    __syncthreads();
    int32_t base = inc - total;
    for (int w = 0; w < wave; w++) base += s_w[w];
    if (d < nb) digit_base[d] = base;
}

__global__ __launch_bounds__(256) void radix_chunk_apply_kernel(const int32_t* __restrict__ hist, int nb, int ntiles,
                                                                const int32_t* __restrict__ chunk_off, const int32_t* __restrict__ digit_base,
                                                                int32_t* __restrict__ offs)
{
    const int t0 = blockIdx.x * SCAN_CHUNK, t1 = min(t0 + SCAN_CHUNK, ntiles);
    for (int d = threadIdx.x; d < nb; d += 256) {
        int32_t run = chunk_off[(int64_t)blockIdx.x * nb + d] + digit_base[d];
#pragma unroll 8
        for (int t = t0; t < t1; t++) {
            const int32_t v = hist[(int64_t)t * nb + d];
            offs[(int64_t)t * nb + d] = run;
            run += v;
        }
    }
}

template <bool RTN>
__device__ __forceinline__ uint32_t wave_rank(uint32_t* cnt, uint32_t digit, int bits, bool valid, int lane)
{
    const uint64_t vm = __ballot(valid);
    if (vm == 0ull) return 0u;
    const int first = __ffsll((long long)vm) - 1;
// ... 107 lines not shown
    }
    if (lane == 63) s_wsum[wave] = inc;
    __syncthreads();
    int32_t run = inc - local;
    for (int w = 0; w < wave; w++) run += s_wsum[w];
#pragma unroll
    for (int k = 0; k < DPT; k++) {
        const int d = threadIdx.x * DPT + k;
        if (d < nb) {
            s_start[d] = (uint16_t)run;
            s_goff[d] = offs[(int64_t)blockIdx.x * nb + d] - run;
        }
        run += tot[k];
    }
    __syncthreads();
#pragma unroll
    for (int r = 0; r < SI; r++) {
        if (base + (int64_t)r * 64 < n) {
            const uint32_t digit = (key[r] >> shift) & mask;
            const int pos = (int)s_start[digit] + (int)c16[wave * NBMAX + digit] + (int)rank[r];
            s_pair[pos] = make_uint2(key[r], idx[r]);
        }
    }
    __syncthreads();
    const int count = (int)((n - tile0) < TILE ? (n - tile0) : TILE);
    for (int j = threadIdx.x; j < count; j += ST) {
        const uint2 v = s_pair[j];
        const int64_t dst = (int64_t)s_goff[(v.x >> shift) & mask] + j;
        if (LAST) idx_out[dst] = v.y;
        else pairs_out[dst] = v;
    }
}

struct SortPlan {
    int npass, bits[4], shift[4];
    int ntiles, nchunks;
    uint2* pbuf[2];
    uint32_t* keys0;
    int32_t *hist, *offs, *chunk_sum, *chunk_off, *digit_base;
    bool fits;
};

size_t sort_layout(void* tmp, size_t bytes, int64_t n, int drop_bits, SortPlan* p)
{
    const int nbits = 30 - drop_bits;
    p->npass = (nbits + MAXB - 1) / MAXB;
    int left = nbits, sh = drop_bits;
    for (int k = 0; k < p->npass; k++) {
        const int b = (left + (p->npass - k) - 1) / (p->npass - k);
        p->bits[k] = b; p->shift[k] = sh; sh += b; left -= b;
    }
    p->ntiles = (int)((n + TILE - 1) / TILE);
    p->nchunks = (p->ntiles + SCAN_CHUNK - 1) / SCAN_CHUNK;
    ia::Carver c(tmp, bytes);
    for (int k = 0; k < 2; k++) {
        p->pbuf[k] = reinterpret_cast<uint2*>(c.take<uint32_t>((size_t)n));
        c.take<uint32_t>((size_t)n);
    }
    p->keys0 = reinterpret_cast<uint32_t*>(p->pbuf[1]);
    p->hist = c.take<int32_t>((size_t)NBMAX * (size_t)p->ntiles);
    p->offs = c.take<int32_t>((size_t)NBMAX * (size_t)p->ntiles);
    p->chunk_sum = c.take<int32_t>((size_t)NBMAX * (size_t)p->nchunks);
    p->chunk_off = c.take<int32_t>((size_t)NBMAX * (size_t)p->nchunks, 4);
    p->digit_base = c.take<int32_t>((size_t)NBMAX, 4);
    c.align_to(256);
    c.skip(256);
    p->fits = c.fits();
    return c.need(256);
}

int g_rank_mode = 0;

}

IA_EXPORT int ia_sort_rank_mode(void) { return g_rank_mode; }

IA_EXPORT size_t ia_morton_order_tmp_bytes(int64_t n)
{
    SortPlan p;
    if (n <= 0) return 256;
    return sort_layout(nullptr, SIZE_MAX, n, 0, &p);
}

IA_EXPORT int ia_morton_order(int64_t n, const float* pts, const float* origin_host3, float inv_cell, int drop_bits, int32_t* order,
                              void* tmp, size_t tmp_bytes, ia_stream_t stream)
{
    if (n == 0) return IA_OK;
    IA_REQUIRE(n < ((int64_t)1 << 31), "ia_morton_order: n must stay below 2^31");
    IA_REQUIRE(drop_bits >= 0 && drop_bits < 30, "ia_morton_order: drop_bits out of range");
    SortPlan p;
    sort_layout(tmp, tmp_bytes, n, drop_bits, &p);
    IA_REQUIRE(tmp != nullptr && p.fits, "ia_morton_order: tmp too small (ia_morton_order_tmp_bytes)");
    IA_REQUIRE((reinterpret_cast<uintptr_t>(tmp) & 255) == 0, "ia_morton_order: tmp must be 256-byte aligned");
    hipStream_t s = (hipStream_t)stream;
    uint2* const* pbuf = p.pbuf;
    uint32_t* keys0 = p.keys0;
    int32_t *hist = p.hist, *offs = p.offs;
    static const int raster = getenv("IA_SORT_RASTER_BITS") ? atoi(getenv("IA_SORT_RASTER_BITS")) : 0;
    const size_t lds = (size_t)2 * TILE * sizeof(uint32_t);
    constexpr int MAX_DEVICES = 64;
    static std::once_flag once[MAX_DEVICES];
    static bool rtn_ok_dev[MAX_DEVICES];
    static int setup_rc[MAX_DEVICES];
    int dev = 0;
    if (hipGetDevice(&dev) != hipSuccess || dev < 0 || dev >= MAX_DEVICES) {
        ia::set_error("ia_morton_order: hipGetDevice failed or device index >= %d", MAX_DEVICES);
        return IA_ERR_LAUNCH;
    }
    std::call_once(once[dev], [lds, dev]() {
        rtn_ok_dev[dev] = false;
        setup_rc[dev] = 0;
#define IA_SET_LDS(F, L, R) if (hipFuncSetAttribute(reinterpret_cast<const void*>(&radix_scatter_kernel<F, L, R>), hipFuncAttributeMaxDynamicSharedMemorySize, (int)lds) != hipSuccess) setup_rc[dev] = 1
        IA_SET_LDS(true, false, true); IA_SET_LDS(false, false, true); IA_SET_LDS(false, true, true); IA_SET_LDS(true, true, true);
        IA_SET_LDS(true, false, false); IA_SET_LDS(false, false, false); IA_SET_LDS(false, true, false); IA_SET_LDS(true, true, false);
#undef IA_SET_LDS
        const char* mode = getenv("IA_SORT_RANK");
        if (mode && !strcmp(mode, "ballot")) return;
        int32_t* d = nullptr;
        int32_t h = -1;
        if (hipMalloc(reinterpret_cast<void**>(&d), sizeof(int32_t)) != hipSuccess) return;
        if (hipMemset(d, 0, sizeof(int32_t)) == hipSuccess) {
            rtn_order_probe_kernel<<<1, 64, 0, 0>>>(2048, d);
            if (hipMemcpy(&h, d, sizeof(int32_t), hipMemcpyDeviceToHost) != hipSuccess) h = -1;
        }
        (void)hipFree(d);
        rtn_ok_dev[dev] = (h == 0);
    });
    if (setup_rc[dev] != 0) {
        (void)hipGetLastError();
        ia::set_error("ia_morton_order: hipFuncSetAttribute(MaxDynamicSharedMemorySize = %zu) failed on device %d", lds, dev);
        return IA_ERR_LAUNCH;
    }
    const bool rtn_ok = rtn_ok_dev[dev];
    g_rank_mode = rtn_ok ? 1 : 2;
    for (int k = 0; k < p.npass; k++) {
        const bool first = k == 0, last = k == p.npass - 1;
        const uint2* pin = first ? nullptr : pbuf[(k - 1) & 1];
        uint2* pout = pbuf[k & 1];
        const int nb = 1 << p.bits[k];
        if (first)
            radix_count_kernel<true><<<p.ntiles, CT, 0, s>>>(n, pts, origin_host3[0], origin_host3[1], origin_host3[2], inv_cell, keys0, nullptr,
                                                             p.shift[k], p.bits[k], hist, p.ntiles, raster);
        else
            radix_count_kernel<false><<<p.ntiles, CT, 0, s>>>(n, nullptr, 0.f, 0.f, 0.f, 0.f, nullptr, pin, p.shift[k], p.bits[k], hist, p.ntiles, 0);
        const int nchunks = p.nchunks;
        int32_t *chunk_sum = p.chunk_sum, *chunk_off = p.chunk_off, *digit_base = p.digit_base;
        radix_chunk_sums_kernel<<<nchunks, 256, 0, s>>>(hist, nb, p.ntiles, chunk_sum);
        radix_chunk_bases_kernel<<<1, 1024, 0, s>>>(chunk_sum, nb, nchunks, chunk_off, digit_base);
        radix_chunk_apply_kernel<<<nchunks, 256, 0, s>>>(hist, nb, p.ntiles, chunk_off, digit_base, offs);
#define IA_SCATTER(F, L, R) radix_scatter_kernel<F, L, R><<<p.ntiles, ST, lds, s>>>(n, keys0, pin, pout, reinterpret_cast<uint32_t*>(order), p.shift[k], p.bits[k], offs, p.ntiles)
        if (rtn_ok) {
            if (first && last) IA_SCATTER(true, true, true); else if (first) IA_SCATTER(true, false, true);
            else if (last) IA_SCATTER(false, true, true); else IA_SCATTER(false, false, true);
        } else {
            if (first && last) IA_SCATTER(true, true, false); else if (first) IA_SCATTER(true, false, false);
            else if (last) IA_SCATTER(false, true, false); else IA_SCATTER(false, false, false);
        }
#undef IA_SCATTER
    }
    return ia::check_launch("ia_morton_order");
}

IA_EXPORT int ia_gather_rows3_i32(int64_t n, const float* src, const int32_t* order, float* dst, ia_stream_t stream)
{
    if (n == 0) return IA_OK;
    gather_rows3_i32_kernel<<<ia::cdiv(n, THREADS), THREADS, 0, (hipStream_t)stream>>>(n, src, order, dst);
    return ia::check_launch("ia_gather_rows3_i32");
}

IA_EXPORT int ia_scatter_f32_i32(int64_t n, const float* src, const int32_t* order, float* dst, ia_stream_t stream)
{
    if (n == 0) return IA_OK;
    scatter_f32_i32_kernel<<<ia::cdiv(n, THREADS), THREADS, 0, (hipStream_t)stream>>>(n, src, order, dst);
    return ia::check_launch("ia_scatter_f32_i32");
}

IA_EXPORT int ia_scatter_rows3_i32(int64_t n, const float* src, const int32_t* order, float* dst, ia_stream_t stream)
{
    if (n == 0) return IA_OK;
    scatter_rows3_i32_kernel<<<ia::cdiv(n, THREADS), THREADS, 0, (hipStream_t)stream>>>(n, src, order, dst);
    return ia::check_launch("ia_scatter_rows3_i32");
}
```

intrinsicavatar_amd/deformer.py:

```python
from typing import Optional

import ctypes as C
import os
import threading

import torch
from torch import Tensor

from . import _lib as L
from . import fast_snarf


class SNARFDeformer:
    INIT_BONES = [0, 1, 2, 4, 5, 10, 11, 12, 15, 16, 17, 18, 19]
    SPEC_EPS = float(os.environ.get("IA_BROYDEN_SPEC_EPS", "1e-3"))
    SPEC_MIN_POINTS = int(os.environ.get("IA_BROYDEN_SPEC_MIN_POINTS", "1"))

    def __init__(self, lbs_voxel_final: Tensor, offset_kernel: Tensor, scale_kernel: Tensor, bbox: Tensor):
        self.lbs_voxel_final = lbs_voxel_final.contiguous().float()
        self.offset_kernel = offset_kernel.reshape(3).contiguous().float()
        self.scale_kernel = scale_kernel.reshape(3).contiguous().float()
        self.bbox = bbox
        self.device = self.lbs_voxel_final.device
        self.init_bones = torch.tensor(self.INIT_BONES, dtype=torch.int32, device=self.device)
# ... 90 lines not shown
        fwd = torch.empty((1, P, I, 3, 3), device=self.device) if want_fwd else None
        if self.spec_eps > 0.0 and P >= self.SPEC_MIN_POINTS and self.tfs.shape[0] == 1:
            fast_snarf.fuse_broyden_spec(x, pts.reshape(1, P, 3), fast_snarf.ChannelLastVoxelJ(self.voxel_J_cl), self.tfs,
                                         self.init_bones, Jinv, valid, self.offset_kernel, self.scale_kernel, 1e-5, 1e-1,
                                         self.spec_eps, fwd_J=fwd, counters=self.spec_counters, cell_tight=self.cell_tight)
        else:
            fast_snarf.fuse_broyden(x, pts.reshape(1, P, 3), None, fast_snarf.ChannelLastVoxelJ(self.voxel_J_cl), self.tfs,
                                    self.init_bones, True, Jinv, valid, self.offset_kernel, self.scale_kernel, 1e-5, 1e-1,
                                    fwd_J=fwd)
        if want_jinv:
            return x[0], valid[0], (fwd[0] if want_fwd else None), Jinv[0]
        return x[0], valid[0], (fwd[0] if want_fwd else None)

    def query_weights(self, xc: Tensor) -> Tensor:
        g = ((xc + self.offset_kernel) * self.scale_kernel).reshape(1, -1, 1, 1, 3)
        w = torch.nn.functional.grid_sample(self.lbs_voxel_final, g, align_corners=True, mode="bilinear",
                                            padding_mode="border")
        return w.reshape(w.shape[1], -1).t()

    def implicit_pose_terms(self, xc: Tensor, J_inv: Tensor, valid: Tensor):
        with torch.no_grad():
            w = self.query_weights(xc)
        T = (w @ self.tfs[0].reshape(w.shape[1], 16)).reshape(-1, 4, 4)
        R = T[:, :3, :3]
        xd = (R * xc[:, None, :]).sum(-1) + T[:, :3, 3]
        corr = -(J_inv * (xd - xd.detach())[:, None, :]).sum(-1)
        corr = corr * valid[:, None].to(corr.dtype)
        return xc + corr, R

    @torch.no_grad()
    def _pack_candidates(self, x: Tensor, valid: Tensor, with_src: bool):
        P, I = valid.shape
        dev = x.device
        lib, st = L.lib(), L.stream()
        cnt = torch.empty(P, dtype=torch.int32, device=dev)
        start = torch.empty(P, dtype=torch.int32, device=dev)
        total = torch.empty(1, dtype=torch.int32, device=dev)
        src = torch.empty(P * I, dtype=torch.int32, device=dev) if with_src else None
        if os.environ.get("IA_PACK", "tiles") == "lookback":
            nbytes = int(lib.ia_deform_filter_compact_tmp_bytes(L.i64(P)))
            tmp = L.work_area(nbytes, dev)
            L.check(lib.ia_deform_filter_compact(L.i64(P), L.i32(I), L.ptr(x), L.ptr(valid), L.ptr(cnt), L.ptr(start), L.ptr(x),
                                                 L.ptr(src), L.ptr(None), L.ptr(total), L.ptr(tmp), C.c_size_t(nbytes), st),
                    "ia_deform_filter_compact")
            Q = int(total.item())
            self._check_voxels()
            return x.reshape(-1, 3)[:Q], (src[:Q] if with_src else None), cnt, start, Q
        nbytes = int(lib.ia_deform_filter_tiles_tmp_bytes(L.i64(P)))
        tmp = L.work_area(nbytes, dev)
        L.check(lib.ia_deform_filter_tiles(L.i64(P), L.i32(I), L.ptr(x), L.ptr(valid), L.ptr(cnt), L.ptr(start), L.ptr(src), L.ptr(None),
                                           L.ptr(total), L.ptr(tmp), C.c_size_t(nbytes), st), "ia_deform_filter_tiles")
        Q = int(total.item())
        self._check_voxels()
        cand_x = torch.empty((Q, 3), device=dev)
        cand_src = torch.empty(Q, dtype=torch.int32, device=dev) if with_src else None
        L.check(lib.ia_deform_pack_tiles(L.i64(P), L.i32(I), L.ptr(x), L.ptr(src), L.ptr(start), L.ptr(cand_x), L.ptr(cand_src),
                                         L.ptr(tmp), st), "ia_deform_pack_tiles")
        return cand_x, cand_src, cnt, start, Q

    SPEC_ROWS = os.environ.get("IA_BROYDEN_SPEC_ROWS", "1") == "1"
    SEARCH_TOKEN = os.environ.get("IA_SEARCH_TOKEN", "0") == "1"
    SEARCH_TOKEN_MIN_POINTS = int(os.environ.get("IA_SEARCH_TOKEN_MIN_POINTS", str(1 << 22)))
    _search_lock = __import__("threading").Lock()
    _search_event = None

    @torch.no_grad()
    def _candidates(self, pts: Tensor, with_src: bool, want_fwd: bool = False, want_jinv: bool = False, order: Optional[Tensor] = None,
                    normalize=None, split: bool = False):
        P, I = pts.shape[0], self.init_bones.shape[0]
        dev = self.device
        if not (self.SPEC_ROWS and self.spec_eps >= 1e-4 and P >= self.SPEC_MIN_POINTS and self.tfs.shape[0] == 1):
            if order is not None:
                pts = pts[order.long()].contiguous()
            r = self.search(pts, want_fwd=want_fwd, want_jinv=want_jinv)
            x, valid, fwd = r[0], r[1], r[2]
            J_inv = r[3] if want_jinv else None
            res = self._normalized((*self._pack_candidates(x, valid, with_src=with_src), fwd, J_inv), normalize)
            return res + (None, None) if split else res
        lib, st = L.lib(), L.stream()
        x_rows = torch.empty((P, 3, 3), device=dev)
        Jinv = torch.empty((1, P, I, 3, 3), device=dev) if want_jinv else None
        fwd = torch.empty((1, P, I, 3, 3), device=dev) if want_fwd else None
        cnt, meta, start, ovf_head = (torch.empty(P, dtype=torch.int32, device=dev) for _ in range(4))
        ovf_scratch = L.work_area(lib.ia_spec_rows_overflow_bytes(L.i64(P)), dev, "spec_rows")
        ovf_cap = self._tls.ovf_cap = int(lib.ia_spec_rows_overflow_capacity(L.i64(P)))
        tot = torch.empty(2, dtype=torch.int32, device=dev)
        token = self.SEARCH_TOKEN and P >= self.SEARCH_TOKEN_MIN_POINTS
        if token:
            self._search_lock.acquire()
        try:
            if token and self._search_event is not None:
                torch.cuda.current_stream(dev).wait_event(self._search_event)
            fast_snarf.fuse_broyden_spec_rows(x_rows, pts.reshape(1, P, 3), fast_snarf.ChannelLastVoxelJ(self.voxel_J_cl), self.tfs, self.init_bones,
                                              Jinv, cnt, meta, start, ovf_head, ovf_scratch, tot, self.offset_kernel, self.scale_kernel,
                                              1e-5, 1e-1, self.spec_eps, fwd_J=fwd, counters=self.spec_counters, order=order,
                                              cell_tight=self.cell_tight)
            if token:
                ev = torch.cuda.Event()
                ev.record(torch.cuda.current_stream(dev))
                type(self)._search_event = ev
        finally:
            if token:
                self._search_lock.release()
        Q, n_over = tot.tolist()
        self._tls.n_over = n_over
        self._check_voxels()
        if os.environ.get("IA_DEBUG_FLAGGED"):
            import sys
            print(f"[spec rows] P={P} Q={Q} redone={n_over} ({n_over / max(P, 1):.2e}) cap={ovf_cap}", file=sys.stderr)
        if n_over > ovf_cap:
            del x_rows, cnt, meta, start, Jinv, fwd
            if order is not None:
                pts = pts[order.long()].contiguous()
            r = self.search(pts, want_fwd=want_fwd, want_jinv=want_jinv)
            res = self._normalized((*self._pack_candidates(r[0], r[1], with_src=with_src), r[2], (r[3] if want_jinv else None)), normalize)
            return res + (None, None) if split else res
        if self.spec_canary > 0:
            self._canary(pts, order, x_rows, cnt, meta)
        cand_x = torch.empty((Q, 3), device=dev)
        if split and not with_src and not want_fwd and not want_jinv and self.SPLIT_CANDIDATES:
            tiles = (P + 1023) // 1024
            first_pos = torch.empty(P, dtype=torch.int32, device=dev)
            tile_off_n = torch.empty(tiles + 1, dtype=torch.int32, device=dev)
            L.check(lib.ia_deform_rows_pack_split(L.i64(P), L.i32(I), L.ptr(x_rows), L.ptr(cnt), L.ptr(meta), L.ptr(start), L.ptr(ovf_head),
                                                  L.ptr(ovf_scratch), L.ptr(first_pos), L.ptr(tile_off_n), L.ptr(tile_off_n[tiles:]), L.ptr(cand_x),
                                                  L.ptr(normalize[0].contiguous().float() if normalize else None),
                                                  L.ptr(normalize[1].contiguous().float() if normalize else None),
                                                  L.ptr(L.work_area(lib.ia_deform_rows_pack_split_tmp_bytes(L.i64(P)), dev)), st), "ia_deform_rows_pack_split")
            return cand_x, None, cnt, start, Q, None, None, (first_pos, tile_off_n[:tiles]), tile_off_n[tiles:]
        cand_src = torch.empty(Q, dtype=torch.int32, device=dev) if with_src else None
        L.check(lib.ia_deform_rows_pack(L.i64(P), L.i32(I), L.ptr(x_rows), L.ptr(cnt), L.ptr(meta), L.ptr(start), L.ptr(ovf_head),
                                        L.ptr(ovf_scratch), L.ptr(cand_x), L.ptr(cand_src),
                                        L.ptr(normalize[0].contiguous().float() if normalize else None),
                                        L.ptr(normalize[1].contiguous().float() if normalize else None), st), "ia_deform_rows_pack")
        res = (cand_x, cand_src, cnt, start, Q, (fwd[0] if want_fwd else None), (Jinv[0] if want_jinv else None))
        return res + (None, None) if split else res

    SPLIT_CANDIDATES = os.environ.get("IA_SPLIT_CANDIDATES", "1") == "1"
    SPEC_CANARY = int(os.environ.get("IA_SPEC_CANARY", "0"))

    @torch.no_grad()
    def _canary(self, pts: Tensor, order: Optional[Tensor], x_rows: Tensor, cnt: Tensor, meta: Tensor):
        P, I = cnt.shape[0], self.init_bones.shape[0]
        dev = pts.device
        k = int(self.spec_canary)
        idx = torch.arange(getattr(self._tls, "canary_phase", 0) % k, P, k, device=dev)
        self._tls.canary_phase = getattr(self._tls, "canary_phase", 0) + 7
        if idx.numel() == 0:
            return
        src = order.long()[idx] if order is not None else idx
        sub = pts[src].contiguous()
        n = sub.shape[0]
        x = torch.empty((1, n, I, 3), device=dev)
        valid = torch.empty((1, n, I), dtype=torch.bool, device=dev)
        fast_snarf.fuse_broyden(x, sub.reshape(1, n, 3), None, fast_snarf.ChannelLastVoxelJ(self.voxel_J_cl), self.tfs, self.init_bones,
                                True, None, valid, self.offset_kernel, self.scale_kernel, 1e-5, 1e-1)
        keep = fast_snarf.filter(x, valid)[0]
        x = x[0]
        c, m, rows = cnt[idx].long(), meta[idx], x_rows[idx]
        flagged = m < 0
        bad = c != keep.sum(1)
        inits = torch.arange(I, device=dev)
        want_bits = (keep.long() << inits[None]).sum(1)
        got_bits = torch.zeros_like(want_bits)
        for j in range(3):
            live = (c > j) & ~flagged
            init = ((m >> (8 * j)) & 0xFF).long().clamp(max=I - 1)
            got_bits = got_bits | torch.where(live, torch.ones_like(c) << init, torch.zeros_like(c))
            ref = torch.gather(x, 1, init[:, None, None].expand(n, 1, 3))[:, 0]
            same = (rows[:, j].view(torch.int32) == ref.view(torch.int32)).all(1)
            bad = bad | (live & ~same)
        bad = bad | (~flagged & (got_bits != want_bits))
        skey = (str(dev), torch.cuda.current_stream(dev).cuda_stream)
        with self._canary_lock:
            acc = self._canary_by_stream.get(skey)
            if acc is None:
                acc = self._canary_by_stream[skey] = torch.zeros(3, dtype=torch.int64, device=dev)
                self._canary_parts.append(acc)
        acc += torch.stack([torch.full((), n, dtype=torch.int64, device=dev), bad.sum(), flagged.sum()])

    def canary_totals(self, reset: bool = False):
        torch.cuda.synchronize(self.device)
        with self._canary_lock:
            tot = [int(v) for v in torch.stack(self._canary_parts).sum(0).tolist()] if self._canary_parts else [0, 0, 0]
            if reset:
                for a in self._canary_parts:
                    a.zero_()
        return tuple(tot)

    @staticmethod
    def _normalized(res, normalize):
        if normalize is None:
            return res
        return ((res[0] - normalize[0]) / normalize[1] + 0.5, *res[1:])

    @torch.no_grad()
    def deform_sdf(self, pts: Tensor, geometry, order: Optional[Tensor] = None) -> Tensor:
        pts = pts.contiguous().float()
        P, I = pts.shape[0], self.init_bones.shape[0]
        dev = self.device
        lib, st = L.lib(), L.stream()
        cand_x, _, cnt, start, Q, _, _, first_pos, n_first = self._candidates(pts, with_src=False, order=order,
                                                                             normalize=(geometry.center, geometry.scale), split=True)
        csdf = geometry.sdf_only(cand_x, normalized=True)
        sdf = torch.empty(P, device=dev)
        if first_pos is not None:
            L.check(lib.ia_deform_select_min_split(L.i64(P), L.ptr(start), L.ptr(cnt), L.ptr(first_pos[0]), L.ptr(first_pos[1]), L.ptr(n_first),
                                                   L.ptr(csdf), L.ptr(order), L.ptr(sdf), st), "ia_deform_select_min_split")
        elif order is not None:
            L.check(lib.ia_deform_select_min_scatter(L.i64(P), L.ptr(start), L.ptr(cnt), L.ptr(csdf), L.ptr(order), L.ptr(sdf), st),
                    "ia_deform_select_min_scatter")
        else:
            L.check(lib.ia_deform_select_min(L.i64(P), L.ptr(start), L.ptr(cnt), L.ptr(csdf), L.ptr(sdf), st), "ia_deform_select_min")
        return sdf

    @torch.no_grad()
    def deform(self, pts: Tensor, geometry, with_grad: bool = False, with_feature: bool = False, want_fwd: bool = False,
               want_jinv: bool = False):
        pts = pts.contiguous().float()
        P, I = pts.shape[0], self.init_bones.shape[0]
        dev = self.device
# ... 37 lines not shown
```

intrinsicavatar_amd/fast_snarf.py:

```python
import torch
from torch import Tensor

from . import _lib as L


class ChannelLastVoxelJ:

    def __init__(self, data: Tensor):
        assert data.dim() == 5 and data.shape[-1] == 12
        self.data = data.contiguous()


def precompute(voxel_w: Tensor, tfs: Tensor, voxel_d: Tensor, voxel_J: Tensor, offset: Tensor, scale: Tensor,
               voxel_J_cl: Tensor = None) -> None:
    B = tfs.shape[0]
    _, C24, D, H, W = voxel_w.shape
    assert C24 == 24 and tfs.shape[1:] == (24, 4, 4)
    voxel_w, tfs = voxel_w.contiguous().float(), tfs.contiguous().float()
    off, sc = offset.reshape(3).contiguous().float(), scale.reshape(3).contiguous().float()
    for t in (voxel_d, voxel_J, voxel_J_cl):
        if t is not None and (not t.is_contiguous() or t.dtype != torch.float32):
            raise RuntimeError("output grids must be contiguous float32")
    L.check(L.lib().ia_precompute(L.i32(B), L.i32(D), L.i32(H), L.i32(W), L.ptr(voxel_w), L.ptr(tfs), L.ptr(off),
                                  L.ptr(sc), L.ptr(voxel_d), L.ptr(voxel_J), L.ptr(voxel_J_cl), L.stream()),
            "ia_precompute")


CELL_TAU = 2.5


def cell_tightness(voxel_J: ChannelLastVoxelJ, offset: Tensor, scale: Tensor, tau: float = CELL_TAU) -> Tensor:
    assert isinstance(voxel_J, ChannelLastVoxelJ) and voxel_J.data.shape[0] == 1
    _, D, H, W, _ = voxel_J.data.shape
    out = torch.empty((D, H, W), dtype=torch.uint8, device=voxel_J.data.device)
    L.check(L.lib().ia_cell_tightness(L.i32(D), L.i32(H), L.i32(W), L.ptr(voxel_J.data), L.ptr(offset.reshape(3).contiguous().float()),
                                      L.ptr(scale.reshape(3).contiguous().float()), L.f32(tau), L.ptr(out), L.stream()), "ia_cell_tightness")
    return out


def _cell_tight_arg(cell_tight, voxel_J):
    if cell_tight is None:
        return None
    if cell_tight.dtype != torch.uint8 or tuple(cell_tight.shape) != tuple(voxel_J.data.shape[1:4]) or not cell_tight.is_contiguous():
        raise RuntimeError("cell_tight must be a contiguous uint8 [D,H,W] tensor (fast_snarf.cell_tightness)")
    return cell_tight


def fuse_broyden(x: Tensor, xd_tgt: Tensor, voxel: Tensor, voxel_J, tfs: Tensor, bone_ids: Tensor,
                 align_corners: bool, J_inv: Tensor, is_valid: Tensor, offset: Tensor, scale: Tensor,
                 cvg_threshold: float, dvg_threshold: float, fwd_J: Tensor = None) -> None:
    B, N, _ = xd_tgt.shape
    I = bone_ids.shape[0]
    if isinstance(voxel_J, ChannelLastVoxelJ):
        vj, layout = voxel_J.data, 1
        _, D, H, W, _ = vj.shape
    else:
        vj, layout = voxel_J.contiguous(), 0
        _, _, D, H, W = vj.shape
    for t in (x, J_inv, is_valid):
        if t is not None and not t.is_contiguous():
            raise RuntimeError("outputs must be contiguous")
    if x.shape != (B, N, I, 3) or (J_inv is not None and J_inv.shape != (B, N, I, 3, 3)) or is_valid.shape != (B, N, I):
        raise RuntimeError("output shapes must be x[B,N,I,3], J_inv[B,N,I,3,3], is_valid[B,N,I]")
    xd = xd_tgt.contiguous().float()
    tfs = tfs.contiguous().float()
    bones = bone_ids.contiguous().to(torch.int32)
    off, sc = offset.reshape(3).contiguous().float(), scale.reshape(3).contiguous().float()
    L.check(L.lib().ia_fuse_broyden(L.i32(B), L.i64(N), L.i32(I), L.ptr(xd), L.ptr(vj), L.i32(layout), L.i32(D),
                                    L.i32(H), L.i32(W), L.ptr(tfs), L.ptr(bones), L.ptr(off), L.ptr(sc),
                                    L.f32(cvg_threshold), L.f32(dvg_threshold), L.ptr(x), L.ptr(J_inv),
                                    L.ptr(is_valid), L.ptr(fwd_J), L.stream()), "ia_fuse_broyden")


def fuse_broyden_spec(x: Tensor, xd_tgt: Tensor, voxel_J: ChannelLastVoxelJ, tfs: Tensor, bone_ids: Tensor, J_inv: Tensor,
                      is_valid: Tensor, offset: Tensor, scale: Tensor, cvg_threshold: float, dvg_threshold: float, eps: float,
                      fwd_J: Tensor = None, counters: Tensor = None, cell_tight: Tensor = None) -> None:
    B, N, _ = xd_tgt.shape
    I = bone_ids.shape[0]
    assert B == 1 and isinstance(voxel_J, ChannelLastVoxelJ) and voxel_J.data.shape[0] == 1
    _, D, H, W, _ = voxel_J.data.shape
    if x.shape != (B, N, I, 3) or (J_inv is not None and J_inv.shape != (B, N, I, 3, 3)) or is_valid.shape != (B, N, I):
        raise RuntimeError("output shapes must be x[B,N,I,3], J_inv[B,N,I,3,3], is_valid[B,N,I]")
    for t in (x, J_inv, is_valid, fwd_J):
        if t is not None and not t.is_contiguous():
            raise RuntimeError("outputs must be contiguous")
    L.check(L.lib().ia_fuse_broyden_spec(
        L.i64(N), L.i32(I), L.ptr(xd_tgt.contiguous().float()), L.ptr(voxel_J.data), L.i32(D), L.i32(H), L.i32(W),
        L.ptr(tfs.contiguous().float()), L.ptr(bone_ids.contiguous().to(torch.int32)), L.ptr(offset.reshape(3).contiguous().float()),
        L.ptr(scale.reshape(3).contiguous().float()), L.f32(cvg_threshold), L.f32(dvg_threshold), L.f32(eps), L.ptr(x), L.ptr(J_inv),
        L.ptr(is_valid), L.ptr(fwd_J), L.ptr(counters), L.ptr(_cell_tight_arg(cell_tight, voxel_J)), L.stream()), "ia_fuse_broyden_spec")


def fuse_broyden_spec_rows(x_rows: Tensor, xd_tgt: Tensor, voxel_J: ChannelLastVoxelJ, tfs: Tensor, bone_ids: Tensor, J_inv: Tensor,
                           cnt: Tensor, meta: Tensor, start: Tensor, ovf_head: Tensor, ovf_scratch: Tensor, total_and_overflow: Tensor,
                           offset: Tensor, scale: Tensor, cvg_threshold: float, dvg_threshold: float, eps: float, fwd_J: Tensor = None,
                           counters: Tensor = None, order: Tensor = None, n_points: int = None, cell_tight: Tensor = None) -> None:
    B, N, _ = xd_tgt.shape
    if order is not None:
        N = order.shape[0]
    I = bone_ids.shape[0]
    assert B == 1 and isinstance(voxel_J, ChannelLastVoxelJ) and voxel_J.data.shape[0] == 1
    _, D, H, W, _ = voxel_J.data.shape
    assert x_rows.shape == (N, 3, 3) and all(t.shape == (N,) and t.dtype == torch.int32 for t in (cnt, meta, start, ovf_head))
    assert total_and_overflow.shape == (2,) and total_and_overflow.dtype == torch.int32
    need = int(L.lib().ia_spec_rows_overflow_bytes(L.i64(N)))
    if ovf_scratch.dtype != torch.uint8 or not ovf_scratch.is_contiguous() or ovf_scratch.numel() < need:
        raise RuntimeError(f"ovf_scratch must be a contiguous uint8 tensor of at least ia_spec_rows_overflow_bytes(N={N}) = {need} bytes "
                           f"(got {ovf_scratch.dtype}, {ovf_scratch.numel()})")
    for t in (x_rows, J_inv, fwd_J, cnt, meta, start):
        if t is not None and not t.is_contiguous():
            raise RuntimeError("outputs must be contiguous")
    L.check(L.lib().ia_fuse_broyden_spec_rows(
        L.i64(N), L.i32(I), L.ptr(xd_tgt.contiguous().float()), L.ptr(voxel_J.data), L.i32(D), L.i32(H), L.i32(W),
        L.ptr(tfs.contiguous().float()), L.ptr(bone_ids.contiguous().to(torch.int32)), L.ptr(offset.reshape(3).contiguous().float()),
        L.ptr(scale.reshape(3).contiguous().float()), L.f32(cvg_threshold), L.f32(dvg_threshold), L.f32(eps), L.ptr(x_rows), L.ptr(J_inv),
        L.ptr(fwd_J), L.ptr(cnt), L.ptr(meta), L.ptr(start), L.ptr(ovf_head), L.ptr(ovf_scratch), L.ptr(total_and_overflow),
        L.ptr(L.scan_tmp(N, xd_tgt.device)), L.ptr(counters), L.ptr(order), L.ptr(_cell_tight_arg(cell_tight, voxel_J)), L.stream()),
        "ia_fuse_broyden_spec_rows")


def filter(x: Tensor, mask: Tensor) -> Tensor:
    B, N, I = mask.shape
    if B != 1:
        raise NotImplementedError("filter: B == 1 only (the reference's index math is only valid for B == 1)")
    x = x.contiguous().float()
    mask = mask.contiguous()
    out = torch.empty_like(mask)
    L.check(L.lib().ia_filter(L.i64(N), L.i32(I), L.ptr(x), L.ptr(mask), L.ptr(out), L.stream()), "ia_filter")
    return out


SMOOTH_SWEEPS = 30
KNN_K = 30


def skin_grid_points(D: int, H: int, W: int, ratio: float, scale: float, offset, device) -> Tensor:
    out = torch.empty((D * H * W, 3), dtype=torch.float32, device=device)
    ox, oy, oz = (float(v) for v in offset)
    L.check(L.lib().ia_skin_grid_points(L.i32(D), L.i32(H), L.i32(W), L.f32(ratio), L.f32(scale), L.f32(ox), L.f32(oy), L.f32(oz),
                                        L.ptr(out), L.stream()), "ia_skin_grid_points")
    return out


def skin_blend(d2: Tensor, idx: Tensor, weights: Tensor) -> Tensor:
    P, K = d2.shape
    if idx.dtype != torch.int32 or idx.shape != d2.shape or weights.dim() != 2 or weights.shape[1] != 24:
        raise RuntimeError("skin_blend: d2 [P,K] fp32, idx [P,K] int32, weights [V,24]")
    out = torch.empty((24, P), dtype=torch.float32, device=d2.device)
    L.check(L.lib().ia_skin_blend(L.i64(P), L.i32(weights.shape[0]), L.i32(K), L.ptr(d2.contiguous().float()), L.ptr(idx.contiguous()),
                                  L.ptr(weights.contiguous().float()), L.ptr(out), L.stream()), "ia_skin_blend")
    return out


def skin_smooth(weights: Tensor, sweeps: int = SMOOTH_SWEEPS) -> Tensor:
    if weights.dim() != 4 or weights.shape[0] != 24:
        raise RuntimeError("skin_smooth: weights [24,D,H,W]")
    _, D, H, W = weights.shape
    a = weights.contiguous().float()
    if sweeps == 0:
        return a
    if a.data_ptr() == weights.data_ptr():
        a = a.clone()
    b = torch.empty_like(a)
    for _ in range(sweeps):
        L.check(L.lib().ia_skin_smooth(L.i32(D), L.i32(H), L.i32(W), L.ptr(a), L.ptr(b), L.stream()), "ia_skin_smooth")
        a, b = b, a
    return a


def query_weights_smpl(x: Tensor, smpl_verts: Tensor, smpl_weights: Tensor, resolution: int = 128) -> Tensor:
    from . import pytorch3d_ops
    d, h, w = resolution // 4, resolution, resolution
    if x.dim() != 3 or x.shape[0] != 1 or x.shape[1] != d * h * w:
        raise ValueError(f"query_weights_smpl: x must be [1, {d * h * w}, 3] for resolution {resolution}, got {tuple(x.shape)}")
    if not x.is_cuda:
        raise L.IaError("query_weights_smpl needs GPU tensors (no CPU fallback)")
    d2, idx = pytorch3d_ops.knn_points_flat(x[0].detach().contiguous().float(), smpl_verts[0].detach().contiguous().float(), KNN_K)
    blend = skin_blend(d2, idx, smpl_weights[0].detach())
    return skin_smooth(blend.view(24, d, h, w), SMOOTH_SWEEPS)[None]
```

intrinsicavatar_amd/render.py:

```python
import os
from typing import Dict, Optional

import torch
from torch import Tensor

from . import _lib as L
from . import lib_nerfacc, nerfacc
from .deformer import SNARFDeformer
from .nerfacc import RayIntervals


def ray_points(rays_o: Tensor, rays_d: Tensor, ray_indices: Tensor, t0: Tensor, t1: Optional[Tensor] = None) -> Tensor:
    n = ray_indices.shape[0]
    pts = torch.empty((n, 3), device=rays_o.device)
    L.check(L.lib().ia_ray_points(L.i64(n), L.ptr(rays_o), L.ptr(rays_d), L.ptr(ray_indices), L.ptr(t0), L.ptr(t1),
                                  L.ptr(pts), L.stream()), "ia_ray_points")
    return pts


def laplace_alpha(sdf: Tensor, dists, beta: Tensor) -> Tensor:
    n = sdf.shape[0]
    alpha = torch.empty_like(sdf)
    d_t, d_c = (dists, 0.0) if isinstance(dists, Tensor) else (None, float(dists))
    L.check(L.lib().ia_laplace_alpha(L.i64(n), L.ptr(sdf), L.ptr(d_t), L.f32(d_c), L.ptr(beta), L.ptr(alpha), L.stream()),
# ... 10 lines not shown

def shade_prep(sdf_grad: Tensor, rays_d: Tensor, ray_indices: Tensor, w2s_rot: Tensor):
    n = sdf_grad.shape[0]
    dev = sdf_grad.device
    ns, nw, rf = (torch.empty((n, 3), device=dev) for _ in range(3))
    L.check(L.lib().ia_shade_prep(L.i64(n), L.ptr(sdf_grad), L.ptr(rays_d), L.ptr(ray_indices), L.ptr(w2s_rot), L.ptr(ns),
                                  L.ptr(nw), L.ptr(rf), L.stream()), "ia_shade_prep")
    return ns, nw, rf


def plan_secondary_chunks(M: int, chunk: int, n_streams: int = 1, min_chunk: int = 1 << 22):
    if M <= 0:
        return []
    if n_streams > 1:
        cmax = max(min(chunk * 5 // 8, -(-M // n_streams)), min_chunk, 1)
        n_chunks = n_streams * (-(-M // (n_streams * cmax)))
        bounds = [M * i // n_chunks for i in range(n_chunks + 1)]
        return [(a, b) for a, b in zip(bounds[:-1], bounds[1:]) if b > a]
    chunk = max(int(chunk), 1)
    return [(c0, min(c0 + chunk, M)) for c0 in range(0, M, chunk)]


class RenderStep:

    def __init__(self, geometry, radiance, density, deformer: SNARFDeformer, occ_binaries: Tensor, occ_aabb: Tensor,
                 render_step_size: float, importance_sample: bool = True):
        self.geometry, self.radiance, self.density, self.deformer = geometry, radiance, density, deformer
        self.binaries, self.aabbs = occ_binaries, occ_aabb
        self._grid_bits = None
        self.render_step_size = float(render_step_size)
        self.importance_sample = importance_sample

    @property
    def grid_bits(self) -> Tensor:
        b = self.binaries
        key = (b.data_ptr(), b._version, str(b.device))
        if self._grid_bits is None or self._grid_bits[0] != key:
            self._grid_bits = (key, nerfacc.pack_occupancy_bits(b[0]))
        return self._grid_bits[1]

    def _beta(self) -> Tensor:
        d = self.density
        return d.beta_value() if hasattr(d, "beta_value") else d.get_beta().detach().reshape(1).float().contiguous()

    _CONST = {}

    @classmethod
    def _const(cls, value: float, n: int, dev) -> Tensor:
        key = (float(value), str(dev), torch.cuda.current_stream(dev).cuda_stream if str(dev).startswith("cuda") else 0)
        t = cls._CONST.get(key)
        if t is None or t.shape[0] < n:
            t = cls._CONST[key] = torch.full((max(n + n // 4, 4096),), float(value), device=dev)
        return t[:n]

    SORT_MIN_POINTS = 1 << 20
    MAX_SEARCH_POINTS = int(os.environ.get("IA_MAX_SEARCH_POINTS", str(150_000_000)))
    K2_MERGED_READBACK = os.environ.get("IA_K2_MERGED_READBACK", "1") == "1"

    SORT_DROP_BITS = int(os.environ.get("IA_SORT_DROP_BITS", "0"))

    def _sort_grid_params(self):
        gkey = (self.aabbs.data_ptr(), self.aabbs._version)
        c = getattr(self, "_sort_grid_cache", None)
        if c is None or c[0] != gkey:
            box = self.aabbs[0].tolist()
            ext = max(box[3] - box[0], box[4] - box[1], box[5] - box[2]) + 0.04
            c = (gkey, [box[0] - 0.02, box[1] - 0.02, box[2] - 0.02], float(os.environ.get("IA_SORT_INV_CELL", 1023.0 / ext)))
            self._sort_grid_cache = c
        return c[1], c[2]

    @torch.no_grad()
    def _spatial_order(self, pts: Tensor) -> Tensor:
        n = pts.shape[0]
        import ctypes as C
        lo, inv_cell = self._sort_grid_params()
        origin = (C.c_float * 3)(*lo)
        lib, st = L.lib(), L.stream()
        order = torch.empty(n, dtype=torch.int32, device=pts.device)
        nb = int(lib.ia_morton_order_tmp_bytes(L.i64(n)))
        tmp = L.work_area(nb, pts.device, "morton")
        L.check(lib.ia_morton_order(L.i64(n), L.ptr(pts), origin, L.f32(inv_cell), L.i32(self.SORT_DROP_BITS), L.ptr(order), L.ptr(tmp),
                                    C.c_size_t(nb), st), "ia_morton_order")
        return order

    @torch.no_grad()
    def _sdf_at(self, pts: Tensor) -> Tensor:
        n = pts.shape[0]
        if n > self.MAX_SEARCH_POINTS:
            return torch.cat([self._sdf_at(pts[a:a + self.MAX_SEARCH_POINTS]) for a in range(0, n, self.MAX_SEARCH_POINTS)])
        if n < self.SORT_MIN_POINTS or os.environ.get("IA_SORT_POINTS", "1") != "1":
            return self.deformer.deform_sdf(pts, self.geometry)
        return self.deformer.deform_sdf(pts, self.geometry, order=self._spatial_order(pts))

    @torch.no_grad()
    def sample(self, rays: Tensor, jitter: Optional[Tensor] = None):
        dfm = self.deformer
        rays = dfm.transform_rays_w2s(rays.float())
        n_rays = rays.shape[0]
        rays_o, rays_d, far = rays[:, 0:3].contiguous(), rays[:, 3:6].contiguous(), rays[:, 7]
        beta = self._beta()
        near_planes = self._const(0.0, n_rays, rays.device)
        far_planes = self._const(1e10, n_rays, rays.device)
        if jitter is not None:
            near_planes = near_planes + jitter * self.render_step_size
        intervals, samples, _ = nerfacc.traverse_grids(rays_o, rays_d, self.binaries, self.aabbs, near_planes, far_planes,
                                                       self.render_step_size, 0.0, grid_bits=self.grid_bits, termination_planes=False)
        stats = dict(n_edges0=intervals.vals.shape[0], n_samples0=samples.vals.shape[0])
        smp_next = None
        if self.importance_sample and samples.vals.numel() > 0:
            for it in range(2):
                vals = intervals.vals
                if it == 0:
                    pts = ray_points(rays_o, rays_d, intervals.ray_indices, vals)
                    sdf = self._sdf_at(pts)
                    sdf_merge = torch.empty_like(sdf)
                    L.check(L.lib().ia_edge_min_sdf(L.i64(sdf.shape[0]), L.ptr(sdf), L.ptr(intervals.is_left), L.ptr(sdf_merge), L.stream()),
                            "ia_edge_min_sdf")
                    alphas = laplace_alpha(sdf_merge, self.render_step_size, beta)
                else:
                    smp = smp_next
                    pts = ray_points(rays_o, rays_d, smp.ray_indices, smp.t_starts, smp.t_ends)
                    sdf_curr = self._sdf_at(pts)
                    alphas = laplace_alpha(smp.to_edges(sdf_curr, 1e10), smp.to_edges(smp.t_ends - smp.t_starts, 0.0), beta)
                weights, _ = nerfacc.render_weight_from_alpha(alphas, packed_info=intervals.packed_info)
                if self.K2_MERGED_READBACK:
                    rvals, ril, rir, ray_idx, pinfo, smp_next = lib_nerfacc.ray_resampling_merge_compact_samples(
                        intervals.packed_info, vals, intervals.is_left, intervals.is_right, weights, 16)
                else:
                    rvals, ril, rir, ray_idx, pinfo = lib_nerfacc.ray_resampling_merge_compact(
                        intervals.packed_info, vals, intervals.is_left, intervals.is_right, weights, 16)
                    smp_next = lib_nerfacc.interval_samples(pinfo, rvals, ril, ray_idx)
                intervals = RayIntervals(vals=rvals, is_left=ril, is_right=rir, ray_indices=ray_idx, packed_info=pinfo)
        smp = smp_next if smp_next is not None else \
            lib_nerfacc.interval_samples(intervals.packed_info, intervals.vals, intervals.is_left, intervals.ray_indices)
        t_starts, t_ends, ray_indices, packed_info = smp.t_starts, smp.t_ends, smp.ray_indices, smp.packed_info
        stats["n_samples"] = t_starts.shape[0]
        return rays_o, rays_d, far, t_starts, t_ends, ray_indices, packed_info, stats

    @torch.no_grad()
    def forward(self, rays: Tensor, jitter: Optional[Tensor] = None) -> Dict[str, Tensor]:
        dfm = self.deformer
        rays_o, rays_d, far, t_starts, t_ends, ray_indices, packed_info, stats = self.sample(rays, jitter)
        beta = self._beta()
        pts = ray_points(rays_o, rays_d, ray_indices, t_starts, t_ends)
        d = dfm.deform(pts, self.geometry, with_grad=True, with_feature=True)
        w2s_rot = dfm.w2s[:3, :3].contiguous()
        normal_smpl, normal_world, refl01 = shade_prep(d["sdf_grad"], rays_d, ray_indices, w2s_rot)
        dists = t_ends - t_starts
        alphas = laplace_alpha(d["sdf"], dists, beta)
        rgbs = self.radiance(d["pts_cano"], d["feature"], refl01, normal_world)
        weights, trans = nerfacc.render_weight_from_alpha(alphas, packed_info=packed_info)
        acc = lambda v: nerfacc._Accumulate.apply(weights, v, ray_indices, packed_info)
        colors, normals, opac = acc(rgbs), acc(normal_world), acc(None)
        depths = acc(((t_starts + t_ends) / 2.0)[:, None])
        depths = depths + (1.0 - opac) * far[:, None]
        stats["n_candidates"] = d["n_candidates"]
        return dict(comp_rgb=colors, comp_normal=normals, opacity=opac, depth=depths, weights=weights, trans=trans,
                    alphas=alphas, rgbs=rgbs, sdf=d["sdf"], sdf_grad=d["sdf_grad"], normals=normal_smpl,
                    positions=d["pts_cano"], valid=d["valid"], t_starts=t_starts, t_ends=t_ends,
                    ray_indices=ray_indices, packed_info=packed_info, stats=stats)

    def parameters(self):
        ps = list(self.geometry.parameters()) + list(self.radiance.parameters()) + list(self.density.parameters())
        return [p for p in ps if p.requires_grad]

    def forward_backward(self, rays: Tensor, target_rgb: Tensor, target_mask: Optional[Tensor] = None,
                         jitter: Optional[Tensor] = None, curv_u: Optional[Tensor] = None, lambda_curv: float = 0.0,
                         loss_scale: float = 1.0, **loss_kw) -> Dict[str, Tensor]:
        from . import train
        rays_o, rays_d, far, t_starts, t_ends, ray_indices, packed_info, stats = self.sample(rays, jitter)
        if curv_u is not None:
            curv_u = curv_u[:t_starts.shape[0]]
        out = train.shade_differentiable(self, rays_o, rays_d, ray_indices, t_starts, t_ends, packed_info, curv_u=curv_u)
        loss = train.training_loss(out, target_rgb, target_mask, lambda_curv=lambda_curv, **loss_kw)
        (loss * loss_scale if loss_scale != 1.0 else loss).backward()
        out["loss"] = loss.detach()
        out["stats"] = stats
        return out

    def forward_backward_phys(self, rays: Tensor, target_rgb: Tensor, material, emitter, spp: int, light_u: Tensor,
                              shuffle_u: Tensor, target_mask: Optional[Tensor] = None, jitter: Optional[Tensor] = None,
                              render_mode: str = "uniform_light", env_base: Optional[Tensor] = None,
                              background_color: Optional[Tensor] = None, global_illumination: bool = False,
                              light_sampling: str = "shared", loss_scale: float = 1.0, retain_graph: bool = False,
                              material_jitter: Optional[Tensor] = None, loss_config: Optional[dict] = None,
                              eik_denominator=None) -> Dict[str, Tensor]:
        from . import train_phys
        rays_o, rays_d, far, t_starts, t_ends, ray_indices, packed_info, stats = self.sample(rays, jitter)
        out = train_phys.shade_differentiable_phys(self, material, emitter, rays_o, rays_d, ray_indices, t_starts, t_ends,
                                                   packed_info, spp, light_u, shuffle_u, render_mode=render_mode,
                                                   env_base=env_base, background_color=background_color,
                                                   global_illumination=global_illumination, light_sampling=light_sampling,
                                                   jitter_n=material_jitter)
        if loss_config is None:
            den = eik_denominator(int(t_starts.shape[0])) if callable(eik_denominator) else eik_denominator
            loss = train_phys.training_loss_phys(out, target_rgb, target_mask, **({} if den is None else dict(eik_denominator=den)))
        else:
            if background_color is None:
                background_color = torch.ones(3, device=rays.device)
            d = self._training_dict(out, rays.shape[0], far, t_starts, t_ends, ray_indices, packed_info, background_color, render_mode)
            loss, out["loss_terms"] = train_phys.reference_training_loss(d, target_rgb, target_mask, loss_config, material)
            out["output_dict"] = d
        (loss * loss_scale if loss_scale != 1.0 else loss).backward(retain_graph=retain_graph)
        out["loss"] = loss.detach()
        out["stats"].update(stats)
# ... 33 lines not shown
                    self._secondary_chunks(my_work, *args)
            except BaseException as e:
                errors.append(e)
        threads = []
        for side, my_work in zip(self._side_streams, works):
            side.wait_stream(main)
            threads.append(threading.Thread(target=worker, args=(side, my_work), daemon=True))
        for t in threads:
            t.start()
        for t in threads:
            t.join()
        for side in self._side_streams:
            main.wait_stream(side)
        if not errors:
            self._side_pool_bytes = n_streams * max(b - a for a, b in chunks) * self.SECONDARY_BYTES_PER_RAY
        if errors:
            if all(isinstance(e, torch.cuda.OutOfMemoryError) for e in errors):
                del errors[:]
                self._side_streams = None
                torch.cuda.synchronize(dev)
                torch.cuda.empty_cache()
                self.secondary_stream_fallbacks = getattr(self, "secondary_stream_fallbacks", 0) + 1
                self._stream_cooldown = self.STREAM_FALLBACK_COOLDOWN
                tr.fill_(1.0)
                rgb.zero_()
                self._secondary_chunks(plan_secondary_chunks(M, chunk, 1)[::-1], *args)
                return tr, rgb
            raise errors[0]
        return tr, rgb

    import threading as _threading
    _march_hooks = _threading.local()
    SECONDARY_STREAMS = int(os.environ.get("IA_SECONDARY_STREAMS", "2"))
    STREAM_FALLBACK_COOLDOWN = int(os.environ.get("IA_STREAM_FALLBACK_COOLDOWN", "64"))
    SECONDARY_BYTES_PER_RAY = int(os.environ.get("IA_SECONDARY_BYTES_PER_RAY", "7168"))

    def _secondary_streams_for(self, M: int, chunk: int, dev) -> int:
        n = getattr(self._march_hooks, "streams", None) or self.SECONDARY_STREAMS
        if n <= 1 or dev.type != "cuda" or M <= self.SECONDARY_STREAMS_MIN_RAYS:
            self.last_secondary_streams = 1
            return 1
        if getattr(self, "_stream_cooldown", 0) > 0:
            self._stream_cooldown -= 1
            self.last_secondary_streams = 1
            return 1
        plan = plan_secondary_chunks(M, chunk, n, self.SECONDARY_MIN_CHUNK)
        in_flight = n * max(b - a for a, b in plan) * self.SECONDARY_BYTES_PER_RAY
        free, _total = torch.cuda.mem_get_info(dev)
        need = 1.3 * in_flight
        have_side = getattr(self, "_side_streams", None) is not None
        if free < need and not (have_side and free + getattr(self, "_side_pool_bytes", 0) >= need):
            side_ids = {st.cuda_stream for st in (getattr(self, "_side_streams", None) or [])}
            side = 0
            if side_ids:
                try:
                    for seg in torch.cuda.memory_snapshot():
                        if seg.get("device", dev.index) == dev.index and seg.get("stream") in side_ids:
                            side += seg["total_size"] - seg["allocated_size"]
                except Exception:
                    side = getattr(self, "_side_pool_bytes", 0)
            n = n if free + side >= need else 1
        self.last_secondary_streams = n
        return n
    SECONDARY_STREAMS_MIN_RAYS = int(os.environ.get("IA_SECONDARY_STREAMS_MIN_RAYS", str(1 << 23)))
    SECONDARY_MIN_CHUNK = int(os.environ.get("IA_SECONDARY_MIN_CHUNK", str(1 << 22)))

    def _secondary_chunks(self, work, rays_o, rays_d, near, far, step, beta, w2s_rot, tr, rgb):
        dev = rays_o.device
        while work:
            c0, c1 = work.pop()
            ro, rd = rays_o[c0:c1].contiguous(), rays_d[c0:c1].contiguous()
            m = ro.shape[0]
            intervals, samples, _ = nerfacc.traverse_grids(
                ro, rd, self.binaries, self.aabbs, self._const(near, m, dev), self._const(far, m, dev),
                step, 0.0, grid_bits=self.grid_bits, max_extent=far - near, incoherent=True, termination_planes=False)
            if samples.vals.shape[0] > 4 * self.MAX_SEARCH_POINTS and m > 1:
                del intervals, samples
                work.extend([(c0 + m // 2, c1), (c0, c0 + m // 2)])
                continue
            t_starts, t_ends = samples.interval_ends(intervals)
            ray_indices = samples.ray_indices
            if t_starts.numel() == 0:
                continue
            sdf = self._sdf_at(ray_points(ro, rd, ray_indices, t_starts))
            alphas = laplace_alpha_intervals(sdf, t_starts, t_ends, beta)
            pinfo = lib_nerfacc.pack_info(ray_indices, m)
            rpi, rs, re, is_fg = lib_nerfacc.ray_resampling_sdf_fine(pinfo, t_starts[:, None], t_ends[:, None], alphas, sdf, 4, exact_size=False)
            ray_indices, t_starts, t_ends, pinfo = lib_nerfacc.compact_foreground(rpi, rs, re, is_fg)
            if t_starts.numel() == 0:
                continue
            pts = ray_points(ro, rd, ray_indices, t_starts, t_ends)
            np_ = pts.shape[0]
            if np_ >= self.SORT_MIN_POINTS and os.environ.get("IA_SORT_POINTS", "1") == "1":
                order = self._spatial_order(pts)
                ps = torch.empty_like(pts)
                L.check(L.lib().ia_gather_rows3_i32(L.i64(np_), L.ptr(pts), L.ptr(order), L.ptr(ps), L.stream()), "ia_gather_rows3_i32")
                ol = order.long()
                ri_s, dt_s = ray_indices[ol], (t_ends - t_starts)[ol]
                d = self.deformer.deform(ps, self.geometry, with_grad=True, with_feature=True)
                _, normal_world, refl01 = shade_prep(d["sdf_grad"], rd, ri_s, w2s_rot)
                a_s = laplace_alpha(d["sdf"], dt_s, beta)
                rgbs_s = self.radiance(d["pts_cano"], d["feature"], refl01, normal_world).contiguous()
                a, rgbs = torch.empty_like(a_s), torch.empty_like(rgbs_s)
                L.check(L.lib().ia_scatter_f32_i32(L.i64(np_), L.ptr(a_s), L.ptr(order), L.ptr(a), L.stream()), "ia_scatter_f32_i32")
                L.check(L.lib().ia_scatter_rows3_i32(L.i64(np_), L.ptr(rgbs_s), L.ptr(order), L.ptr(rgbs), L.stream()), "ia_scatter_rows3_i32")
            else:
                d = self.deformer.deform(pts, self.geometry, with_grad=True, with_feature=True)
                _, normal_world, refl01 = shade_prep(d["sdf_grad"], rd, ray_indices, w2s_rot)
                a = laplace_alpha_intervals(d["sdf"], t_starts, t_ends, beta)
                rgbs = self.radiance(d["pts_cano"], d["feature"], refl01, normal_world)
            w, _ = nerfacc.render_weight_from_alpha(a, packed_info=pinfo)
            acc = nerfacc._Accumulate.apply(w, None, ray_indices, pinfo)
            torch.neg(acc, out=tr[c0:c0 + m])
            tr[c0:c0 + m].add_(1.0)
            rgb[c0:c0 + m] = nerfacc._Accumulate.apply(w, rgbs, ray_indices, pinfo)

    @torch.no_grad()
    def relight(self, rays: Tensor, material, emitter, spp: int, light_u: Tensor, shuffle_u: Tensor,
                background_color: Optional[Tensor] = None, global_illumination: bool = False,
                jitter: Optional[Tensor] = None, render_mode: str = "light", scatter_u: Optional[Tensor] = None,
                return_index_lists: bool = False, albedo_only: bool = False, albedo_align_ratio: Optional[Tensor] = None) -> Dict[str, Tensor]:
        from . import pbr
        dfm = self.deformer
        rays_o, rays_d, far, t_starts, t_ends, ray_indices, packed_info, stats = self.sample(rays, jitter)
        n_rays = rays_o.shape[0]
        dev = rays_o.device
        beta = self._beta()
        w2s_rot = dfm.w2s[:3, :3].contiguous()
        if background_color is None:
            background_color = torch.ones(3, device=dev)
        pts = ray_points(rays_o, rays_d, ray_indices, t_starts, t_ends)
        d = dfm.deform(pts, self.geometry, with_grad=True, with_feature=True)
        normal_smpl, normal_world, refl01 = shade_prep(d["sdf_grad"], rays_d, ray_indices, w2s_rot)
        alphas = laplace_alpha_intervals(d["sdf"], t_starts, t_ends, beta)
        rgbs, enc2, xp2 = self.radiance(d["pts_cano"], d["feature"], refl01, normal_world, return_embedding=True)
        mats = material(enc2, xp2, d["feature"], self.radiance.prog.mask(self.radiance.global_step, dev))
        if albedo_align_ratio is not None:
            mats = torch.cat([mats[:, :3] * albedo_align_ratio.as_subclass(Tensor).to(mats).reshape(1, 3), mats[:, 3:]], dim=1)
        weights, trans = nerfacc.render_weight_from_alpha(alphas, packed_info=packed_info)
        acc = lambda v: nerfacc._Accumulate.apply(weights, v, ray_indices, packed_info)
        out = dict(comp_rgb=acc(rgbs), comp_normal=acc(normal_world), albedo=acc(mats[:, :3].contiguous()),
                   roughness=acc(mats[:, 3:4].contiguous()), metallic=acc(mats[:, 4:5].contiguous()), opacity=acc(None))
        out["depth"] = acc(((t_starts + t_ends) / 2.0)[:, None]) + (1.0 - out["opacity"]) * far[:, None]
        out["packed_info"] = packed_info
        out["primary_samples"] = dict(sdf_grad=d["sdf_grad"], valid=d["valid"], t_starts=t_starts, t_ends=t_ends, ray_indices=ray_indices)
        extras = dict(weights=weights, sdf=d["sdf"], alphas=alphas, normals=normal_smpl, albedo=mats[:, :3],
                      roughness=mats[:, 3:4], metallic=mats[:, 4:5])
        rgb_phys = background_color[None].expand(n_rays, 3).clone()
        demod_phys = rgb_phys.clone()
        if render_mode == "uniform_light":
            out["visibility"] = torch.zeros((n_rays, 1), device=dev)
        stats.update(n_resampled=0, n_fg=0, n_secondary=0)
        if ray_indices.numel() > 0 and not albedo_only:
            vi = pbr.VolumeInteraction(ray_indices, t_starts, t_ends, n_rays, spp, weights, d["sdf"])
            stats["n_resampled"], stats["n_fg"] = vi.R, vi.F
            transmittance = 1.0 - out["opacity"]
            if vi.F > 0:
                F_ = vi.F
                w_fg, nrm, alb, rough, metal = vi.gather(rays_o, rays_d, weights, normal_smpl, mats[:, :3], mats[:, 3:4], mats[:, 4:5])
                pos, view = vi.positions, vi.view_dirs
                ind = lambda c: c if global_illumination else None
                if render_mode in ("light", "uniform_light"):
                    if render_mode == "light":
                        dirs_smpl = emitter.sample(spp, light_u, w2s_rot=w2s_rot)
                        inv_pdf_all = None
                    else:
                        assert spp == 512, "uniform_light asserts samples_per_pixel == 512 (:1392)"
                        dirs_smpl, inv_pdf_all = pbr.uniform_sphere_stratified(16, 32, light_u[:, :2])
                    shuffled = vi.shuffle(shuffle_u)
                    ro, rd, src, out_dirs = pbr.secondary_rays(nrm, pos, dirs_smpl, dir_index=shuffled)
                    inv_pdf = inv_pdf_all[shuffled.long()] if render_mode == "uniform_light" else None
                    stats["n_secondary"] = int(ro.shape[0])
                    t_, c_ = self.compute_indirect_radiance(ro, rd)
                    sec_tr, sec_rgb = pbr.scatter_secondary(F_, src, t_, c_)
                    res = pbr.pbr_shade(render_mode, nrm, alb, rough, metal, view, out_dirs, sec_tr, ind(sec_rgb), emitter, w2s_rot,
                                        inv_pdf=inv_pdf)
                    fg_Lo, fg_demod = res[0], res[1] + res[2]
                    out["shuffled"] = shuffled
                    if render_mode == "uniform_light":
                        zero3 = torch.zeros(3, device=dev)
                        out["visibility"] = vi.composite(w_fg, res[3], torch.zeros_like(transmittance), zero3).mean(-1, keepdim=True)
                elif render_mode in ("mats", "mis"):
                    assert scatter_u is not None and scatter_u.shape[0] >= F_, "mats / mis need scatter_u [n_fg, 6]"
                    sc_dirs = pbr.brdf_sample(nrm, view, rough, scatter_u[:F_, :3])
                    if render_mode == "mis":
                        li_dirs = emitter.sample(F_, scatter_u[:F_, 3:6].contiguous(), w2s_rot=w2s_rot)
                        out_dirs = torch.cat([sc_dirs, li_dirs], 0)
                        rep = lambda t: t.repeat(2, 1)
                    else:
# ... 105 lines not shown
```

Before: 1.005 million.

## Fuse ray-point generation into Morton sort and add fused candidate scan

Computes ray sample points inside the first radix-count pass of the Morton sort, so there is no separate ray_points kernel followed by a key kernel. Replaces the generic exclusive scan plus split-pack prefix with a dedicated three-kernel candidate scan that produces both the candidate starts and the first-occurrence offsets in one pass. It also routes the coarse SDF queries through the spatially sorted path. This cuts kernel launches and redundant passes over memory, at the cost of more code paths gated by environment flags. The ray point math disables FMA contraction so the fused and unfused paths give bitwise-identical points.

```diff
diff --git a/include/ia_amd.h b/include/ia_amd.h
--- a/include/ia_amd.h
+++ b/include/ia_amd.h
@@ -161,6 +161,11 @@
 int ia_deform_rows_pack_split(int64_t N, int I, const float* x_rows, const int32_t* cnt, const uint32_t* meta, const int32_t* start,
                               const int32_t* ovf_head, const void* ovf_scratch, int32_t* first_pos, int32_t* first_tile_off, int32_t* n_first,
                               float* cand_x, const float* norm_center, const float* norm_scale, void* scan_tmp, ia_stream_t stream);
+int ia_candidate_scan(int64_t N, const int32_t* cnt, const void* ovf_scratch , int32_t* start, int32_t* total_and_overflow,
+                      int32_t* first_pos, int32_t* first_tile_off, int32_t* n_first, void* tmp, ia_stream_t stream);
+int ia_deform_rows_pack_scanned(int64_t N, int I, const float* x_rows, const int32_t* cnt, const uint32_t* meta, const int32_t* start,
+                                const int32_t* ovf_head, const void* ovf_scratch, const int32_t* first_pos, const int32_t* first_tile_off,
+                                const int32_t* n_first, float* cand_x, const float* norm_center, const float* norm_scale, ia_stream_t stream);
 int ia_deform_select_min_split(int64_t P, const int32_t* start, const int32_t* cnt, const int32_t* first_pos, const int32_t* first_tile_off,
                                const int32_t* n_first, const float* cand_sdf, const int32_t* order, float* sdf, ia_stream_t stream);
 int ia_broyden_stats(int B, int64_t N, int I, const float* xd_tgt, const float* voxel_J, int layout, int D, int H, int W,
@@ -357,6 +362,9 @@
 size_t ia_morton_order_tmp_bytes(int64_t n);
 int ia_morton_order(int64_t n, const float* pts , const float* origin_host3, float inv_cell, int drop_bits,
                     int32_t* order , void* tmp, size_t tmp_bytes, ia_stream_t stream);
+int ia_ray_points_morton_order(int64_t n, const float* rays_o, const float* rays_d, const int64_t* ray_indices, const float* t0,
+                               const float* t1 , const float* origin_host3, float inv_cell, int drop_bits,
+                               float* pts , int32_t* order , void* tmp, size_t tmp_bytes, ia_stream_t stream);
 int ia_gather_rows3_i32(int64_t n, const float* src, const int32_t* order, float* dst, ia_stream_t stream);
 int ia_scatter_f32_i32(int64_t n, const float* src, const int32_t* order, float* dst, ia_stream_t stream);
 int ia_scatter_rows3_i32(int64_t n, const float* src , const int32_t* order, float* dst ,
diff --git a/intrinsicavatar_amd/csrc/deform.hip b/intrinsicavatar_amd/csrc/deform.hip
--- a/intrinsicavatar_amd/csrc/deform.hip
+++ b/intrinsicavatar_amd/csrc/deform.hip
@@ -1,4 +1,5 @@
 #include "ia_common.h"
+#include "ray_point.h"
 
 namespace {
 
@@ -367,11 +368,11 @@
 {
     const int64_t i = (int64_t)blockIdx.x * THREADS + threadIdx.x;
     if (i >= n) return;
-    const int64_t r = ray_indices[i];
-    const float t = t1 ? (t0[i] + t1[i]) / 2.0f : t0[i];
-    pts[i * 3 + 0] = rays_o[r * 3 + 0] + rays_d[r * 3 + 0] * t;
-    pts[i * 3 + 1] = rays_o[r * 3 + 1] + rays_d[r * 3 + 1] * t;
-    pts[i * 3 + 2] = rays_o[r * 3 + 2] + rays_d[r * 3 + 2] * t;
+    float p[3];
+    ia_ray_point(rays_o, rays_d, ray_indices, t0, t1, i, p);
+    pts[i * 3 + 0] = p[0];
+    pts[i * 3 + 1] = p[1];
+    pts[i * 3 + 2] = p[2];
 }
 
 __device__ __forceinline__ void normalize3(float v[3], float eps)
diff --git a/intrinsicavatar_amd/csrc/ray_point.h b/intrinsicavatar_amd/csrc/ray_point.h
--- /dev/null
+++ b/intrinsicavatar_amd/csrc/ray_point.h
@@ -0,0 +1,18 @@
+#pragma once
+#include <stdint.h>
+
+#include <hip/hip_runtime.h>
+
+__device__ __forceinline__ void ia_ray_point(const float* __restrict__ rays_o, const float* __restrict__ rays_d,
+                                             const int64_t* __restrict__ ray_indices, const float* __restrict__ t0,
+                                             const float* __restrict__ t1, int64_t i, float out[3])
+{
+#pragma clang fp contract(off)
+    const int64_t r = ray_indices[i];
+    const float t = t1 ? (t0[i] + t1[i]) / 2.0f : t0[i];
+#pragma unroll
+    for (int k = 0; k < 3; k++) {
+        const float step = rays_d[r * 3 + k] * t;
+        out[k] = rays_o[r * 3 + k] + step;
+    }
+}
diff --git a/intrinsicavatar_amd/csrc/snarf.hip b/intrinsicavatar_amd/csrc/snarf.hip
--- a/intrinsicavatar_amd/csrc/snarf.hip
+++ b/intrinsicavatar_amd/csrc/snarf.hip
@@ -1089,6 +1089,121 @@
 #pragma unroll
     for (int k = 0; k < 4; k++) { if (base + k < N) first_local[base + k] = run; run += v[k]; }
     if (threadIdx.x == 255) tile_sums[blockIdx.x] = run;
+}
+
+__device__ __forceinline__ void cand_load4(int64_t N, const int32_t* __restrict__ cnt, int64_t base, bool vec, int v[4])
+{
+    if (vec && base + 3 < N) {
+        const int4 q = *reinterpret_cast<const int4*>(cnt + base);
+        v[0] = q.x; v[1] = q.y; v[2] = q.z; v[3] = q.w;
+    } else {
+#pragma unroll
+        for (int k = 0; k < 4; k++) v[k] = base + k < N ? cnt[base + k] : 0;
+    }
+}
+
+__global__ __launch_bounds__(256) void cand_tile_sums_kernel(int64_t N, const int32_t* __restrict__ cnt, int32_t* __restrict__ sum_cnt,
+                                                              int32_t* __restrict__ sum_first, bool vec)
+{
+    __shared__ int s_c[4], s_f[4];
+    const int lane = threadIdx.x & 63, wave = threadIdx.x >> 6;
+    const int64_t base = (int64_t)blockIdx.x * FIRST_TILE + (int64_t)threadIdx.x * 4;
+    int v[4], c = 0, f = 0;
+    cand_load4(N, cnt, base, vec, v);
+#pragma unroll
+    for (int k = 0; k < 4; k++) { c += v[k]; f += v[k] > 0 ? 1 : 0; }
+#pragma unroll
+    for (int off = 32; off > 0; off >>= 1) { c += __shfl_xor(c, off, 64); f += __shfl_xor(f, off, 64); }
+    if (lane == 0) { s_c[wave] = c; s_f[wave] = f; }
+    __syncthreads();
+    if (threadIdx.x == 0) {
+        sum_cnt[blockIdx.x] = s_c[0] + s_c[1] + s_c[2] + s_c[3];
+        sum_first[blockIdx.x] = s_f[0] + s_f[1] + s_f[2] + s_f[3];
+    }
+}
+
+__global__ __launch_bounds__(1024) void cand_tile_bases_kernel(int64_t tiles, int32_t* __restrict__ tile_start ,
+                                                                int32_t* __restrict__ first_tile_off ,
+                                                                int32_t* __restrict__ total, int32_t* __restrict__ n_first,
+                                                                const int32_t* __restrict__ ovf_counts, int ovf_cap, int flag_cap,
+                                                                int32_t* __restrict__ report)
+{
+    __shared__ int s_c[16], s_f[16];
+    __shared__ int carry_c, carry_f;
+    const int tid = threadIdx.x, lane = tid & 63, wave = tid >> 6;
+    if (tid == 0) { carry_c = 0; carry_f = 0; }
+    __syncthreads();
+    for (int64_t chunk = 0; chunk < tiles; chunk += 4096) {
+        const int64_t base = chunk + (int64_t)tid * 4;
+        int vc[4], vf[4], lc = 0, lf = 0;
+#pragma unroll
+        for (int k = 0; k < 4; k++) {
+            vc[k] = base + k < tiles ? tile_start[base + k] : 0;
+            vf[k] = base + k < tiles ? first_tile_off[base + k] : 0;
+            lc += vc[k]; lf += vf[k];
+        }
+        int ic = lc, jf = lf;
+#pragma unroll
+        for (int off = 1; off < 64; off <<= 1) {
+            const int oc = __shfl_up(ic, off, 64), of = __shfl_up(jf, off, 64);
+            if (lane >= off) { ic += oc; jf += of; }
+        }
+        if (lane == 63) { s_c[wave] = ic; s_f[wave] = jf; }
+        __syncthreads();
+        int rc = carry_c + ic - lc, rf = carry_f + jf - lf, tc = 0, tf = 0;
+#pragma unroll
+        for (int w = 0; w < 16; w++) {
+            const int a = s_c[w], b = s_f[w];
+            if (w < wave) { rc += a; rf += b; }
+            tc += a; tf += b;
+        }
+#pragma unroll
+        for (int k = 0; k < 4; k++) {
+            if (base + k < tiles) { tile_start[base + k] = rc; first_tile_off[base + k] = rf; }
+            rc += vc[k]; rf += vf[k];
+        }
+        __syncthreads();
+        if (tid == 0) { carry_c += tc; carry_f += tf; }
+        __syncthreads();
+    }
+    if (tid == 0) {
+        *total = carry_c;
+        *n_first = carry_f;
+        if (ovf_counts) *report = ovf_counts[0] > ovf_cap ? flag_cap + 1 : ovf_counts[1];
+    }
+}
+
+__global__ __launch_bounds__(256) void cand_tile_scan_kernel(int64_t N, const int32_t* __restrict__ cnt, const int32_t* __restrict__ tile_start,
+                                                              int32_t* __restrict__ start, int32_t* __restrict__ first_local, bool vec)
+{
+    __shared__ int s_c[4], s_f[4];
+    const int lane = threadIdx.x & 63, wave = threadIdx.x >> 6;
+    const int64_t base = (int64_t)blockIdx.x * FIRST_TILE + (int64_t)threadIdx.x * 4;
+    int v[4], lc = 0, lf = 0;
+    cand_load4(N, cnt, base, vec, v);
+#pragma unroll
+    for (int k = 0; k < 4; k++) { lc += v[k]; lf += v[k] > 0 ? 1 : 0; }
+    int ic = lc, jf = lf;
+#pragma unroll
+    for (int off = 1; off < 64; off <<= 1) {
+        const int oc = __shfl_up(ic, off, 64), of = __shfl_up(jf, off, 64);
+        if (lane >= off) { ic += oc; jf += of; }
+    }
+    if (lane == 63) { s_c[wave] = ic; s_f[wave] = jf; }
+    __syncthreads();
+    int rc = tile_start[blockIdx.x] + ic - lc, rf = jf - lf;
+    for (int w = 0; w < wave; w++) { rc += s_c[w]; rf += s_f[w]; }
+    int oc[4], of[4];
+#pragma unroll
+    for (int k = 0; k < 4; k++) { oc[k] = rc; of[k] = rf; rc += v[k]; rf += v[k] > 0 ? 1 : 0; }
+    if (vec && base + 3 < N) {
+        *reinterpret_cast<int4*>(start + base) = make_int4(oc[0], oc[1], oc[2], oc[3]);
+        *reinterpret_cast<int4*>(first_local + base) = make_int4(of[0], of[1], of[2], of[3]);
+    } else {
+#pragma unroll
+        for (int k = 0; k < 4; k++)
+            if (base + k < N) { start[base + k] = oc[k]; first_local[base + k] = of[k]; }
+    }
 }
 
 template <int LAYOUT>
@@ -1566,7 +1681,7 @@
     ovf_layout(ovf_scratch, N, &o);
     ia::zero_bytes(o.count, 2 * sizeof(int32_t), s);
     if (N == 0) {
-        ia::zero_bytes(total_and_overflow, 2 * sizeof(int32_t), s);
+        if (start != nullptr) ia::zero_bytes(total_and_overflow, 2 * sizeof(int32_t), s);
         return ia::check_launch("ia_fuse_broyden_spec_rows");
     }
     int64_t small_max = (int64_t)1 << 18;
@@ -1590,6 +1705,7 @@
     r = ia::check_launch("ia_fuse_broyden_spec_rows(flagged)");
     if (r != IA_OK) return r;
     if (small) zero_i32_kernel<<<1, 64, 0, s>>>(o.flag.count);
+    if (start == nullptr) return ia::check_launch("ia_fuse_broyden_spec_rows(flagged)");
     r = ia_exclusive_scan_i32(cnt, start, total_and_overflow, N, scan_tmp, stream);
     if (r != IA_OK) return r;
     rows_report_kernel<<<1, 64, 0, s>>>(o.count, o.flag.cap, total_and_overflow + 1);
@@ -1639,6 +1755,44 @@
     return ia::check_launch("ia_deform_rows_pack_split");
 }
 
+IA_EXPORT int ia_candidate_scan(int64_t N, const int32_t* cnt, const void* ovf_scratch, int32_t* start, int32_t* total_and_overflow,
+                                int32_t* first_pos, int32_t* first_tile_off, int32_t* n_first, void* tmp, ia_stream_t stream)
+{
+    IA_REQUIRE(N >= 0 && N < ((int64_t)1 << 31), "ia_candidate_scan: 0 <= N < 2^31");
+    IA_REQUIRE(total_and_overflow != nullptr && n_first != nullptr, "ia_candidate_scan: total_and_overflow and n_first are required");
+    IA_REQUIRE(N == 0 || (cnt && start && first_pos && first_tile_off && tmp), "ia_candidate_scan: cnt, start, first_pos, first_tile_off and tmp are required");
+    hipStream_t s = (hipStream_t)stream;
+    PackSplitTmp t;
+    pack_split_layout(tmp, N, &t);
+    OvfLayout o;
+    o.count = nullptr;
+    o.flag.cap = 0;
+    if (ovf_scratch) ovf_layout(const_cast<void*>(ovf_scratch), N, &o);
+    const bool vec = ((reinterpret_cast<uintptr_t>(cnt) | reinterpret_cast<uintptr_t>(start) | reinterpret_cast<uintptr_t>(first_pos)) & 15) == 0;
+    if (t.tiles > 0) cand_tile_sums_kernel<<<(int)t.tiles, 256, 0, s>>>(N, cnt, t.sums, first_tile_off, vec);
+    cand_tile_bases_kernel<<<1, 1024, 0, s>>>(t.tiles, t.sums, first_tile_off, total_and_overflow, n_first, o.count, SPEC_OVF_CAP, o.flag.cap,
+                                              total_and_overflow + 1);
+    if (t.tiles > 0) cand_tile_scan_kernel<<<(int)t.tiles, 256, 0, s>>>(N, cnt, t.sums, start, first_pos, vec);
+    return ia::check_launch("ia_candidate_scan");
+}
+
+IA_EXPORT int ia_deform_rows_pack_scanned(int64_t N, int I, const float* x_rows, const int32_t* cnt, const uint32_t* meta, const int32_t* start,
+                                          const int32_t* ovf_head, const void* ovf_scratch, const int32_t* first_pos,
+                                          const int32_t* first_tile_off, const int32_t* n_first, float* cand_x, const float* norm_center,
+                                          const float* norm_scale, ia_stream_t stream)
+{
+    if (N == 0) return IA_OK;
+    IA_REQUIRE(cand_x != x_rows, "ia_deform_rows_pack_scanned: cand_x must not alias x_rows");
+    IA_REQUIRE((norm_center == nullptr) == (norm_scale == nullptr), "ia_deform_rows_pack_scanned: norm_center and norm_scale go together");
+    IA_REQUIRE(first_pos != nullptr && first_tile_off != nullptr && n_first != nullptr,
+               "ia_deform_rows_pack_scanned: first_pos, first_tile_off and n_first are required");
+    OvfLayout o;
+    ovf_layout(const_cast<void*>(ovf_scratch), N, &o);
+    rows_pack_kernel<<<ia::cdiv(N, THREADS), THREADS, 0, (hipStream_t)stream>>>(N, I, x_rows, cnt, meta, start, ovf_head, o.rec, o.x, o.keep, cand_x,
+                                                                                nullptr, norm_center, norm_scale, first_pos, first_tile_off, n_first);
+    return ia::check_launch("ia_deform_rows_pack_scanned");
+}
+
 IA_EXPORT int ia_filter(int64_t N, int I, const float* x, const uint8_t* mask, uint8_t* out, ia_stream_t stream)
 {
     if (N == 0) return IA_OK;
diff --git a/intrinsicavatar_amd/csrc/sort.hip b/intrinsicavatar_amd/csrc/sort.hip
--- a/intrinsicavatar_amd/csrc/sort.hip
+++ b/intrinsicavatar_amd/csrc/sort.hip
@@ -3,6 +3,7 @@
 #include <mutex>
 
 #include "ia_common.h"
+#include "ray_point.h"
 
 namespace {
 
@@ -59,9 +60,9 @@
 constexpr int CT = 256;
 constexpr int CI = TILE / CT;
 
-__device__ __forceinline__ uint32_t morton_key(const float* __restrict__ pts, int64_t i, float ox, float oy, float oz, float inv_cell, int raster = 0)
-{
-    const float fx = (pts[3 * i] - ox) * inv_cell, fy = (pts[3 * i + 1] - oy) * inv_cell, fz = (pts[3 * i + 2] - oz) * inv_cell;
+__device__ __forceinline__ uint32_t morton_key_xyz(float px, float py, float pz, float ox, float oy, float oz, float inv_cell, int raster = 0)
+{
+    const float fx = (px - ox) * inv_cell, fy = (py - oy) * inv_cell, fz = (pz - oz) * inv_cell;
     const uint32_t x = (uint32_t)fminf(fmaxf(fx, 0.0f), 1023.0f), y = (uint32_t)fminf(fmaxf(fy, 0.0f), 1023.0f),
                    z = (uint32_t)fminf(fmaxf(fz, 0.0f), 1023.0f);
     if (raster > 0) {
@@ -72,6 +73,18 @@
     return spread10(x) | (spread10(y) << 1) | (spread10(z) << 2);
 }
 
+__device__ __forceinline__ uint32_t morton_key(const float* __restrict__ pts, int64_t i, float ox, float oy, float oz, float inv_cell, int raster = 0)
+{
+    return morton_key_xyz(pts[3 * i], pts[3 * i + 1], pts[3 * i + 2], ox, oy, oz, inv_cell, raster);
+}
+
+struct RaySrc {
+    const float *rays_o, *rays_d;
+    const int64_t* ray_indices;
+    const float *t0, *t1;
+    float* pts_out;
+};
+
 __device__ __forceinline__ uint64_t digit_peers(uint32_t digit, int bits, bool valid)
 {
     uint64_t peers = __ballot(valid);
@@ -83,10 +96,11 @@
     return peers;
 }
 
-template <bool FIRST>
+template <bool FIRST, bool RAYS = false>
 __global__ __launch_bounds__(CT) void radix_count_kernel(int64_t n, const float* __restrict__ pts, float ox, float oy, float oz, float inv_cell,
                                                           uint32_t* __restrict__ keys , const uint2* __restrict__ pairs ,
-                                                          int shift, int bits, int32_t* __restrict__ hist, int ntiles, int raster)
+                                                          int shift, int bits, int32_t* __restrict__ hist, int ntiles, int raster,
+                                                          RaySrc rays = RaySrc{})
 {
     __shared__ int32_t s_hist[NBMAX];
     const int nb = 1 << bits;
@@ -102,7 +116,13 @@
             const int64_t i = base + (int64_t)(r0 + r) * CT;
             key[r] = 0;
             if (i < n) {
-                if (FIRST) { key[r] = morton_key(pts, i, ox, oy, oz, inv_cell, raster); keys[i] = key[r]; }
+                if (FIRST && RAYS) {
+                    float p[3];
+                    ia_ray_point(rays.rays_o, rays.rays_d, rays.ray_indices, rays.t0, rays.t1, i, p);
+                    rays.pts_out[3 * i] = p[0]; rays.pts_out[3 * i + 1] = p[1]; rays.pts_out[3 * i + 2] = p[2];
+                    key[r] = morton_key_xyz(p[0], p[1], p[2], ox, oy, oz, inv_cell, raster);
+                    keys[i] = key[r];
+                } else if (FIRST) { key[r] = morton_key(pts, i, ox, oy, oz, inv_cell, raster); keys[i] = key[r]; }
                 else key[r] = pairs[i].x;
             }
         }
@@ -376,8 +396,8 @@
     return sort_layout(nullptr, SIZE_MAX, n, 0, &p);
 }
 
-IA_EXPORT int ia_morton_order(int64_t n, const float* pts, const float* origin_host3, float inv_cell, int drop_bits, int32_t* order,
-                              void* tmp, size_t tmp_bytes, ia_stream_t stream)
+static int morton_order_impl(int64_t n, const float* pts, const RaySrc* rays, const float* origin_host3, float inv_cell, int drop_bits,
+                             int32_t* order, void* tmp, size_t tmp_bytes, ia_stream_t stream)
 {
     if (n == 0) return IA_OK;
     IA_REQUIRE(n < ((int64_t)1 << 31), "ia_morton_order: n must stay below 2^31");
@@ -432,7 +452,10 @@
         const uint2* pin = first ? nullptr : pbuf[(k - 1) & 1];
         uint2* pout = pbuf[k & 1];
         const int nb = 1 << p.bits[k];
-        if (first)
+        if (first && rays)
+            radix_count_kernel<true, true><<<p.ntiles, CT, 0, s>>>(n, nullptr, origin_host3[0], origin_host3[1], origin_host3[2], inv_cell, keys0,
+                                                                   nullptr, p.shift[k], p.bits[k], hist, p.ntiles, raster, *rays);
+        else if (first)
             radix_count_kernel<true><<<p.ntiles, CT, 0, s>>>(n, pts, origin_host3[0], origin_host3[1], origin_host3[2], inv_cell, keys0, nullptr,
                                                              p.shift[k], p.bits[k], hist, p.ntiles, raster);
         else
@@ -455,6 +478,21 @@
     return ia::check_launch("ia_morton_order");
 }
 
+IA_EXPORT int ia_morton_order(int64_t n, const float* pts, const float* origin_host3, float inv_cell, int drop_bits, int32_t* order,
+                              void* tmp, size_t tmp_bytes, ia_stream_t stream)
+{
+    return morton_order_impl(n, pts, nullptr, origin_host3, inv_cell, drop_bits, order, tmp, tmp_bytes, stream);
+}
+
+IA_EXPORT int ia_ray_points_morton_order(int64_t n, const float* rays_o, const float* rays_d, const int64_t* ray_indices, const float* t0,
+                                         const float* t1, const float* origin_host3, float inv_cell, int drop_bits, float* pts,
+                                         int32_t* order, void* tmp, size_t tmp_bytes, ia_stream_t stream)
+{
+    IA_REQUIRE(n == 0 || (rays_o && rays_d && ray_indices && t0 && pts), "ia_ray_points_morton_order: rays_o, rays_d, ray_indices, t0 and pts are required");
+    const RaySrc rays = {rays_o, rays_d, ray_indices, t0, t1, pts};
+    return morton_order_impl(n, nullptr, &rays, origin_host3, inv_cell, drop_bits, order, tmp, tmp_bytes, stream);
+}
+
 IA_EXPORT int ia_gather_rows3_i32(int64_t n, const float* src, const int32_t* order, float* dst, ia_stream_t stream)
 {
     if (n == 0) return IA_OK;
diff --git a/intrinsicavatar_amd/deformer.py b/intrinsicavatar_amd/deformer.py
--- a/intrinsicavatar_amd/deformer.py
+++ b/intrinsicavatar_amd/deformer.py
@@ -196,6 +196,7 @@
         Jinv = torch.empty((1, P, I, 3, 3), device=dev) if want_jinv else None
         fwd = torch.empty((1, P, I, 3, 3), device=dev) if want_fwd else None
         cnt, meta, start, ovf_head = (torch.empty(P, dtype=torch.int32, device=dev) for _ in range(4))
+        fused_scan = split and not with_src and not want_fwd and not want_jinv and self.SPLIT_CANDIDATES and self.FUSED_CANDIDATE_SCAN
         ovf_scratch = L.work_area(lib.ia_spec_rows_overflow_bytes(L.i64(P)), dev, "spec_rows")
         ovf_cap = self._tls.ovf_cap = int(lib.ia_spec_rows_overflow_capacity(L.i64(P)))
         tot = torch.empty(2, dtype=torch.int32, device=dev)
@@ -206,9 +207,16 @@
             if token and self._search_event is not None:
                 torch.cuda.current_stream(dev).wait_event(self._search_event)
             fast_snarf.fuse_broyden_spec_rows(x_rows, pts.reshape(1, P, 3), fast_snarf.ChannelLastVoxelJ(self.voxel_J_cl), self.tfs, self.init_bones,
-                                              Jinv, cnt, meta, start, ovf_head, ovf_scratch, tot, self.offset_kernel, self.scale_kernel,
-                                              1e-5, 1e-1, self.spec_eps, fwd_J=fwd, counters=self.spec_counters, order=order,
+                                              Jinv, cnt, meta, None if fused_scan else start, ovf_head, ovf_scratch, tot, self.offset_kernel,
+                                              self.scale_kernel, 1e-5, 1e-1, self.spec_eps, fwd_J=fwd, counters=self.spec_counters, order=order,
                                               cell_tight=self.cell_tight)
+            if fused_scan:
+                tiles = (P + 1023) // 1024
+                first_pos = torch.empty(P, dtype=torch.int32, device=dev)
+                tile_off_n = torch.empty(tiles + 1, dtype=torch.int32, device=dev)
+                L.check(lib.ia_candidate_scan(L.i64(P), L.ptr(cnt), L.ptr(ovf_scratch), L.ptr(start), L.ptr(tot), L.ptr(first_pos), L.ptr(tile_off_n),
+                                              L.ptr(tile_off_n[tiles:]), L.ptr(L.work_area(lib.ia_deform_rows_pack_split_tmp_bytes(L.i64(P)), dev)), st),
+                        "ia_candidate_scan")
             if token:
                 ev = torch.cuda.Event()
                 ev.record(torch.cuda.current_stream(dev))
@@ -224,6 +232,7 @@
             print(f"[spec rows] P={P} Q={Q} redone={n_over} ({n_over / max(P, 1):.2e}) cap={ovf_cap}", file=sys.stderr)
         if n_over > ovf_cap:
             del x_rows, cnt, meta, start, Jinv, fwd
+            first_pos = tile_off_n = None
             if order is not None:
                 pts = pts[order.long()].contiguous()
             r = self.search(pts, want_fwd=want_fwd, want_jinv=want_jinv)
@@ -232,6 +241,12 @@
         if self.spec_canary > 0:
             self._canary(pts, order, x_rows, cnt, meta)
         cand_x = torch.empty((Q, 3), device=dev)
+        if fused_scan:
+            L.check(lib.ia_deform_rows_pack_scanned(L.i64(P), L.i32(I), L.ptr(x_rows), L.ptr(cnt), L.ptr(meta), L.ptr(start), L.ptr(ovf_head),
+                                                    L.ptr(ovf_scratch), L.ptr(first_pos), L.ptr(tile_off_n), L.ptr(tile_off_n[tiles:]), L.ptr(cand_x),
+                                                    L.ptr(normalize[0].contiguous().float() if normalize else None),
+                                                    L.ptr(normalize[1].contiguous().float() if normalize else None), st), "ia_deform_rows_pack_scanned")
+            return cand_x, None, cnt, start, Q, None, None, (first_pos, tile_off_n[:tiles]), tile_off_n[tiles:]
         if split and not with_src and not want_fwd and not want_jinv and self.SPLIT_CANDIDATES:
             tiles = (P + 1023) // 1024
             first_pos = torch.empty(P, dtype=torch.int32, device=dev)
@@ -251,6 +266,7 @@
         return res + (None, None) if split else res
 
     SPLIT_CANDIDATES = os.environ.get("IA_SPLIT_CANDIDATES", "1") == "1"
+    FUSED_CANDIDATE_SCAN = os.environ.get("IA_FUSED_CANDIDATE_SCAN", "1") == "1"
     SPEC_CANARY = int(os.environ.get("IA_SPEC_CANARY", "0"))
 
     @torch.no_grad()
diff --git a/intrinsicavatar_amd/fast_snarf.py b/intrinsicavatar_amd/fast_snarf.py
--- a/intrinsicavatar_amd/fast_snarf.py
+++ b/intrinsicavatar_amd/fast_snarf.py
@@ -101,7 +101,7 @@
     I = bone_ids.shape[0]
     assert B == 1 and isinstance(voxel_J, ChannelLastVoxelJ) and voxel_J.data.shape[0] == 1
     _, D, H, W, _ = voxel_J.data.shape
-    assert x_rows.shape == (N, 3, 3) and all(t.shape == (N,) and t.dtype == torch.int32 for t in (cnt, meta, start, ovf_head))
+    assert x_rows.shape == (N, 3, 3) and all(t.shape == (N,) and t.dtype == torch.int32 for t in (cnt, meta, ovf_head) + (() if start is None else (start,)))
     assert total_and_overflow.shape == (2,) and total_and_overflow.dtype == torch.int32
     need = int(L.lib().ia_spec_rows_overflow_bytes(L.i64(N)))
     if ovf_scratch.dtype != torch.uint8 or not ovf_scratch.is_contiguous() or ovf_scratch.numel() < need:
@@ -115,7 +115,7 @@
         L.ptr(tfs.contiguous().float()), L.ptr(bone_ids.contiguous().to(torch.int32)), L.ptr(offset.reshape(3).contiguous().float()),
         L.ptr(scale.reshape(3).contiguous().float()), L.f32(cvg_threshold), L.f32(dvg_threshold), L.f32(eps), L.ptr(x_rows), L.ptr(J_inv),
         L.ptr(fwd_J), L.ptr(cnt), L.ptr(meta), L.ptr(start), L.ptr(ovf_head), L.ptr(ovf_scratch), L.ptr(total_and_overflow),
-        L.ptr(L.scan_tmp(N, xd_tgt.device)), L.ptr(counters), L.ptr(order), L.ptr(_cell_tight_arg(cell_tight, voxel_J)), L.stream()),
+        L.ptr(L.scan_tmp(N, xd_tgt.device) if start is not None else None), L.ptr(counters), L.ptr(order), L.ptr(_cell_tight_arg(cell_tight, voxel_J)), L.stream()),
         "ia_fuse_broyden_spec_rows")
 
 
diff --git a/intrinsicavatar_amd/render.py b/intrinsicavatar_amd/render.py
--- a/intrinsicavatar_amd/render.py
+++ b/intrinsicavatar_amd/render.py
@@ -116,6 +116,38 @@
         L.check(lib.ia_morton_order(L.i64(n), L.ptr(pts), origin, L.f32(inv_cell), L.i32(self.SORT_DROP_BITS), L.ptr(order), L.ptr(tmp),
                                     C.c_size_t(nb), st), "ia_morton_order")
         return order
+
+    FUSED_POINT_KEYS = os.environ.get("IA_FUSED_POINT_KEYS", "1") == "1"
+
+    def _sorts(self, n: int) -> bool:
+        return self.SORT_MIN_POINTS <= n <= self.MAX_SEARCH_POINTS and os.environ.get("IA_SORT_POINTS", "1") == "1"
+
+    @torch.no_grad()
+    def _ray_points_spatial_order(self, rays_o: Tensor, rays_d: Tensor, ray_indices: Tensor, t0: Tensor, t1: Optional[Tensor] = None):
+        n = ray_indices.shape[0]
+        if not self.FUSED_POINT_KEYS:
+            pts = ray_points(rays_o, rays_d, ray_indices, t0, t1)
+            return pts, self._spatial_order(pts)
+        import ctypes as C
+        lo, inv_cell = self._sort_grid_params()
+        origin = (C.c_float * 3)(*lo)
+        lib, st = L.lib(), L.stream()
+        dev = rays_o.device
+        pts = torch.empty((n, 3), device=dev)
+        order = torch.empty(n, dtype=torch.int32, device=dev)
+        nb = int(lib.ia_morton_order_tmp_bytes(L.i64(n)))
+        tmp = L.work_area(nb, dev, "morton")
+        L.check(lib.ia_ray_points_morton_order(L.i64(n), L.ptr(rays_o), L.ptr(rays_d), L.ptr(ray_indices), L.ptr(t0), L.ptr(t1), origin,
+                                               L.f32(inv_cell), L.i32(self.SORT_DROP_BITS), L.ptr(pts), L.ptr(order), L.ptr(tmp),
+                                               C.c_size_t(nb), st), "ia_ray_points_morton_order")
+        return pts, order
+
+    @torch.no_grad()
+    def _sdf_at_samples(self, rays_o: Tensor, rays_d: Tensor, ray_indices: Tensor, t0: Tensor, t1: Optional[Tensor] = None) -> Tensor:
+        if not self._sorts(ray_indices.shape[0]):
+            return self._sdf_at(ray_points(rays_o, rays_d, ray_indices, t0, t1))
+        pts, order = self._ray_points_spatial_order(rays_o, rays_d, ray_indices, t0, t1)
+        return self.deformer.deform_sdf(pts, self.geometry, order=order)
 
     @torch.no_grad()
     def _sdf_at(self, pts: Tensor) -> Tensor:
@@ -145,16 +177,14 @@
             for it in range(2):
                 vals = intervals.vals
                 if it == 0:
-                    pts = ray_points(rays_o, rays_d, intervals.ray_indices, vals)
-                    sdf = self._sdf_at(pts)
+                    sdf = self._sdf_at_samples(rays_o, rays_d, intervals.ray_indices, vals)
                     sdf_merge = torch.empty_like(sdf)
                     L.check(L.lib().ia_edge_min_sdf(L.i64(sdf.shape[0]), L.ptr(sdf), L.ptr(intervals.is_left), L.ptr(sdf_merge), L.stream()),
                             "ia_edge_min_sdf")
                     alphas = laplace_alpha(sdf_merge, self.render_step_size, beta)
                 else:
                     smp = smp_next
-                    pts = ray_points(rays_o, rays_d, smp.ray_indices, smp.t_starts, smp.t_ends)
-                    sdf_curr = self._sdf_at(pts)
+                    sdf_curr = self._sdf_at_samples(rays_o, rays_d, smp.ray_indices, smp.t_starts, smp.t_ends)
                     alphas = laplace_alpha(smp.to_edges(sdf_curr, 1e10), smp.to_edges(smp.t_ends - smp.t_starts, 0.0), beta)
                 weights, _ = nerfacc.render_weight_from_alpha(alphas, packed_info=intervals.packed_info)
                 if self.K2_MERGED_READBACK:
@@ -354,17 +384,16 @@
             ray_indices = samples.ray_indices
             if t_starts.numel() == 0:
                 continue
-            sdf = self._sdf_at(ray_points(ro, rd, ray_indices, t_starts))
+            sdf = self._sdf_at_samples(ro, rd, ray_indices, t_starts)
             alphas = laplace_alpha_intervals(sdf, t_starts, t_ends, beta)
             pinfo = lib_nerfacc.pack_info(ray_indices, m)
             rpi, rs, re, is_fg = lib_nerfacc.ray_resampling_sdf_fine(pinfo, t_starts[:, None], t_ends[:, None], alphas, sdf, 4, exact_size=False)
             ray_indices, t_starts, t_ends, pinfo = lib_nerfacc.compact_foreground(rpi, rs, re, is_fg)
             if t_starts.numel() == 0:
                 continue
-            pts = ray_points(ro, rd, ray_indices, t_starts, t_ends)
-            np_ = pts.shape[0]
+            np_ = t_starts.shape[0]
             if np_ >= self.SORT_MIN_POINTS and os.environ.get("IA_SORT_POINTS", "1") == "1":
-                order = self._spatial_order(pts)
+                pts, order = self._ray_points_spatial_order(ro, rd, ray_indices, t_starts, t_ends)
                 ps = torch.empty_like(pts)
                 L.check(L.lib().ia_gather_rows3_i32(L.i64(np_), L.ptr(pts), L.ptr(order), L.ptr(ps), L.stream()), "ia_gather_rows3_i32")
                 ol = order.long()
@@ -377,6 +406,7 @@
                 L.check(L.lib().ia_scatter_f32_i32(L.i64(np_), L.ptr(a_s), L.ptr(order), L.ptr(a), L.stream()), "ia_scatter_f32_i32")
                 L.check(L.lib().ia_scatter_rows3_i32(L.i64(np_), L.ptr(rgbs_s), L.ptr(order), L.ptr(rgbs), L.stream()), "ia_scatter_rows3_i32")
             else:
+                pts = ray_points(ro, rd, ray_indices, t_starts, t_ends)
                 d = self.deformer.deform(pts, self.geometry, with_grad=True, with_feature=True)
                 _, normal_world, refl01 = shade_prep(d["sdf_grad"], rd, ray_indices, w2s_rot)
                 a = laplace_alpha_intervals(d["sdf"], t_starts, t_ends, beta)
```

Result: no change. 1.008 million (median of 6 runs) (+0.3%).
